# smann95/mpmc

Measured on AMD Instinct MI355X. Metric: MC steps/sec (polarizable, 4096 atoms), higher is better.
Workload: dtype f64; 1 GPU; PCN-61 cell + 416 BSSP H2, 4096 atoms (2016 frozen), polarizable, Jacobi x4, rc 8 A, FH4; energy() incremental (bit-identical to full); n_atoms=4096, n_polarizable=3264, n_atoms_final=4096, n_polarizable_final=3264, walkers=1, parallelism=1 independent walkers, 1 per GPU, collective=none (single walker, no launcher), rccl_ranks=1

## Files before the change

include/mpmc_hip.h:

```cpp
#ifndef MPMC_HIP_H
#define MPMC_HIP_H

#include <stddef.h>
#include <stdint.h>

#ifdef __cplusplus
extern "C" {
#endif

#define MPMC_HIP_ABI_VERSION 1

typedef struct mpmc_hip_ctx mpmc_hip_ctx;
typedef struct mpmc_hip_comm mpmc_hip_comm;

typedef struct mpmc_hip_params {
    double temperature;
    int rd_only;
    int rd_lrc;
    int feynman_hibbs;
    int feynman_hibbs_order;
    int ewald_alpha_set;
    double ewald_alpha;
    int ewald_kmax;
    int polarization;
// ... 18 lines not shown

typedef struct mpmc_hip_result {
    double energy;
    double rd_energy;
    double coulombic_energy;
    double polarization_energy;
    double es_real, es_recip, es_self;
    double dipole_rrms;
    double volume, cutoff, ewald_alpha, polar_ewald_alpha;
    int polar_iterations;
    int iter_success;
    int n_atoms;
    int status;
} mpmc_hip_result;

typedef struct mpmc_hip_timings {
    float pair_ms;
    float recip_ms;
    float field_ms;
    float amatrix_ms;
    float sweep_ms;
    float palmo_ms;
    float other_ms;
    float total_ms;
    int sweep_count;
    int amatrix_count;
    int graph_steps;
    float event_pair_ms;
    int event_pair_count;
    int spec_rank_redos;
    int resident_calls;
    int resident_fallbacks;
    int pending_sweeps;
} mpmc_hip_timings;

const char *mpmc_hip_last_error(void);
int mpmc_hip_abi_version(void);
int mpmc_hip_device_count(void);

int mpmc_hip_create(mpmc_hip_ctx **ctx, int device, int max_atoms);
void mpmc_hip_destroy(mpmc_hip_ctx *ctx);

int mpmc_hip_set_option(mpmc_hip_ctx *ctx, const char *name, int value);

void mpmc_hip_default_params(mpmc_hip_params *p);
int mpmc_hip_set_params(mpmc_hip_ctx *ctx, const mpmc_hip_params *p);

int mpmc_hip_set_box(mpmc_hip_ctx *ctx, const double basis[9], double pbc_cutoff);

int mpmc_hip_scale_box(mpmc_hip_ctx *ctx, const double basis[9], double pbc_cutoff,
                       int n_molecules, const double *delta );

int mpmc_hip_upload(mpmc_hip_ctx *ctx, int n, const double *x, const double *y, const double *z,
                    const double *charge, const double *polarizability, const double *epsilon,
                    const double *sigma, const double *mass, const int *molecule, const uint8_t *frozen);

typedef struct mpmc_hip_disp_params {
    int disp_expansion;
    int damp_dispersion;
    int extrapolate_disp_coeffs;
    int schmidt_mixing;
} mpmc_hip_disp_params;

int mpmc_hip_set_dispersion(mpmc_hip_ctx *ctx, const mpmc_hip_disp_params *p, int n, const double *c6, const double *c8,
                            const double *c10);

// ... 40 lines not shown
int mpmc_hip_cavity_bin(mpmc_hip_ctx *ctx, int n, const double *x, const double *y, const double *z);
int mpmc_hip_cavity_update(mpmc_hip_ctx *ctx, int n_out, const double *out_xyz, int n_in, const double *in_xyz,
                           int n_darts, const double *dart_xyz, int *cavities_open, int *hits);
int mpmc_hip_cavity_point(mpmc_hip_ctx *ctx, int index, int *grid_index, double pos[3]);
int mpmc_hip_download_cavity_grid(mpmc_hip_ctx *ctx, int *occupancy, double *pos);

int mpmc_hip_update_atoms(mpmc_hip_ctx *ctx, int first, int count, const double *x, const double *y,
                          const double *z);

int mpmc_hip_insert_molecule(mpmc_hip_ctx *ctx, int count, const double *x, const double *y, const double *z,
                             const double *charge, const double *polarizability, const double *epsilon,
                             const double *sigma, const double *mass, int frozen, int *first_slot);
int mpmc_hip_remove_molecule(mpmc_hip_ctx *ctx, int first_slot, int count);

typedef struct {
    int count;
    int frozen;
    const double *x, *y, *z, *charge, *polarizability, *epsilon, *sigma, *mass;
    const double *c6, *c8, *c10;
    const double *c9;
} mpmc_hip_molecule;

int mpmc_hip_edit_molecules(mpmc_hip_ctx *ctx,
                            int nremove, const int *remove_first_slot, const int *remove_count,
                            int ninsert, const mpmc_hip_molecule *insert, int *insert_first_slot);
int mpmc_hip_set_sweep_order(mpmc_hip_ctx *ctx, int count, const int *slots);
int mpmc_hip_slot_count(mpmc_hip_ctx *ctx);

int mpmc_hip_energy(mpmc_hip_ctx *ctx, mpmc_hip_result *out);

int mpmc_hip_energy_begin(mpmc_hip_ctx *ctx);
int mpmc_hip_energy_end(mpmc_hip_ctx *ctx, mpmc_hip_result *out);

int mpmc_hip_download_dipoles(mpmc_hip_ctx *ctx, double *mu, double *ef_static, double *ef_induced,
                              double *ef_induced_change);

int mpmc_hip_download_amatrix(mpmc_hip_ctx *ctx, double *A);

int mpmc_hip_download_ranking(mpmc_hip_ctx *ctx, double *rank_metric, int *ranked_array);

int mpmc_hip_get_timings(mpmc_hip_ctx *ctx, mpmc_hip_timings *t);

int mpmc_hip_comm_unique_id(unsigned char id[128]);
int mpmc_hip_comm_create(mpmc_hip_comm **comm, mpmc_hip_ctx *ctx, int nranks, int rank,
                         const unsigned char id[128]);
int mpmc_hip_comm_size(const mpmc_hip_comm *comm);
int mpmc_hip_comm_rank(const mpmc_hip_comm *comm);
int mpmc_hip_allreduce_observables(mpmc_hip_comm *comm, double *values, int count);
int mpmc_hip_allreduce_observables_begin(mpmc_hip_comm *comm, const double *values, int count);
int mpmc_hip_allreduce_observables_end(mpmc_hip_comm *comm, double *values);
int mpmc_hip_gather_observables(mpmc_hip_comm *comm, const void *record, int bytes, void *records);
void mpmc_hip_comm_destroy(mpmc_hip_comm *comm);

#ifdef __cplusplus
}
#endif
#endif
```

mpmc_amd/csrc/device_common.h:

```cpp
#pragma once
#include <hip/hip_runtime.h>
#include <stdint.h>

#include "step_pods.h"

namespace mpmc {

constexpr double kHBAR2 = 1.11211999e-68;
constexpr double kHBAR4 = 1.23681087e-136;
constexpr double kKB = 1.3806503e-23;
constexpr double kKB2 = 1.90619525e-46;
constexpr double kM2A2 = 1.0e20;
constexpr double kM2A4 = 1.0e40;
constexpr double kAMU2KG = 1.66053873e-27;
constexpr double kDEBYE2SKA = 85.10597636;
constexpr double kMAXVALUE = 1.0e40;
constexpr double kSMALL_dR = 1.0e-12;
constexpr int kMAX_ITERATION_COUNT = 128;
constexpr double kPI = 3.14159265358979323846;
constexpr double kOneOverSqrtPi = 0.56418958354;

constexpr int kWave = 64;

enum AtomFlag : int { kFrozen = 1, kValid = 2 };

struct DevBox {
    double b[3][3];
    double rb[3][3];
    double cutoff;
    double volume;
    float fb[3][3];
    float frb[3][3];
    float rc2_pre;
    int screen64;
    float half_tie32;
    double tie64;
    int tie_guard;
};

constexpr int kMaxMoves = 32;
struct MoveList {
    int n;
    int idx[kMaxMoves];
    double x[kMaxMoves], y[kMaxMoves], z[kMaxMoves];
};
struct MoveTargets {
    double *x, *y, *z;
    const int *slot_of_atom;
    double *px, *py, *pz;
};

struct DevAtoms {
    const double *x, *y, *z;
    const double *q, *alpha, *eps, *sig, *molmass;
    const int *mol;
    const int *flags;
    int n, npad;
};

__device__ __forceinline__ void moved_position(const DevAtoms &a, const MoveList &m, int i, double &x, double &y,
                                               double &z) {
    x = a.x[i];
    y = a.y[i];
    z = a.z[i];
    for (int e = 0; e < m.n; ++e) {
        if (m.idx[e] == i) {
            x = m.x[e];
            y = m.y[e];
            z = m.z[e];
        }
    }
}

__device__ __forceinline__ void minimum_image(const DevBox &bx, double dx, double dy, double dz, double &r,
                                              double &rimg, double &ox, double &oy, double &oz) {
#pragma clang fp contract(off)
    double i0 = bx.rb[0][0] * dx;
    i0 = i0 + bx.rb[1][0] * dy;
// ... 154 lines not shown
```

mpmc_amd/csrc/engine.hip:

```cpp
#include "../../include/mpmc_hip.h"

#include <dlfcn.h>
#include <hip/hip_runtime.h>
#include <hip/hip_ext.h>
#include <rccl/rccl.h>

#include <algorithm>
#include <cmath>
#include <cstdarg>
#include <cstdio>
#include <cstring>
#include <map>
#include <memory>
#include <tuple>
#include <utility>
#include <ctime>
#include <numeric>
#include <atomic>
#include <string>
#include <vector>

#include "device_common.h"
#include "step_plan.h"
#include "kernels_pair.h"
// ... 216 lines not shown
    int timing_interval = 32;
    int persistent_gs = 1;
    int spec_rank = 1;
    int fuse_tensor = 1;
    int gs_lags = 3;
    int gs_build_fork = 1;
    int gs_side_waves = 0;
    int rank_view_side = 1;
    int gs_fold_upper = 1;
    int gs_fold_finish = 1;
    int rank_late = 1;
    int resident = 1;
    int res_fold = 16;
    int res_side = 0;
    int sweep_alternate = 1;
    int sweep_nt = -1;
    int sweep_split = -1;
    int fuse_moves = 1;
    int gs_fuse_moves = 1;
    int fuse_field = 1;
    int fuse_recip = 1;
    int split_record = 1;
    int side_moves = 1;
    int res_stamps = 0;
    int sweep_ablate = 0;
    int res_fault = 0;
    int gs_stamps = 0;
    int inv_stamps = 0;
    int gs_ablate = 0;
    int gs_fault_sweep = 0;
    int graph = 0;
};

struct CallState {
    bool do_polar = false;
    bool gs_mode = false;
    bool exact = false;
    bool two_streams = false;
    bool plain_launches = false;
    DirtyBlocks dirty_blocks;
    DirtyBlocks lrc_blocks;
    bool lrc_edited = false;
    bool pair_part_valid_before = false;
    bool moves_deferred = false;
    bool moves_in_pair = false;
    bool side_carry = false;
    MoveList side_moves;
    MoveList pair_moves;
    MoveList side_apply;
    bool side_applied = false;
    bool coef_job_valid = false;
    bool coef_job_fork = false;
    CoefJob coef_job;
    bool build_join_pending = false;
    bool rank_on_side = false;
    int gs_sweeps = 0;
    bool gs_used[2] = {false, false};
    bool polar_first = false;
    bool side_open = false;
    bool side_done = false;
    int side_rc = 0;
    bool may_publish_early = false;
    bool published = false;
    int publish_rc = 0;
    bool recip_fused = false;
    int recip_chunks = 0;
    int pair_rows_to_sum = 0;
    unsigned res_zero_mask = 0;
    bool split = false;
    bool resident = false;
    bool spec_rank = false;
    bool timed = false;
    int iterations = 0, iter_success = 0;
};

struct TileSum {
    DevBuf<double> part;
    bool valid = false;
};

struct mpmc_hip_ctx {
    int device = 0;
    int num_cus = 256;
    int max_atoms = 0, max_npad = 0;
    int n = 0, npad = 0;
    EngineOptions opt;
// ... 120 lines not shown
    DevBuf<double> d_recipsum;
    bool self_valid = false;
    double self_alpha = 0.0;
    DevBuf<KVecF> d_kvecf;
    DevBuf<double2> d_sf;
    int nkf = 0;
    double kvecf_alpha = -1.0;
    int kvecf_kmax = -1;
    bool kvecf_valid = false;
    DevBuf<double> d_rank;
    DevBuf<double> d_rankpart;
    DevBuf<double> d_rank_used;
    DevBuf<unsigned int> d_rankcnt;
    std::vector<double> rank_saved;
    bool perm_ranked = false;
    bool rank_used_valid = false;
    bool force_host_rank = false;
    unsigned long long spec_redos = 0;
    int n_valid = 0;
    int next_mol = 0;
    std::vector<char> slot_valid;
    std::vector<char> slot_polar;
    std::vector<std::pair<int, int>> holes;
    std::vector<int> lrc_dirty_atoms;
    int n_mol_uploaded = 0;
    bool edited = false;
    bool order_stale = false;
    bool resident_off = false;
    long resident_retry_at = 0;
    long resident_backoff = 0;
    bool force_multi_launch = false;
    bool res_attr_set = false;
    unsigned long long resident_calls = 0, resident_fallbacks = 0;
    int graph_mode = 0;
    StepGraph sg;
    int eligible_streak = 0;
    unsigned long long graph_launches = 0;
    double graph_update_s = 0.0, graph_launch_s = 0.0;
    PinnedBuf<int> h_dirty;
    PinnedBuf<double> h_stage;
    size_t stage_used = 0;
    DevBuf<double> d_delta;
    DevBuf<double> d_res;
    PinnedBuf<double> h_res;
    double *h_res_dev = nullptr;
    PinnedBuf<double> h_res2;
    double *h_res2_dev = nullptr;
    PinnedBuf<unsigned long long> h_err;
    PinnedBuf<unsigned> h_gserr;
    PinnedBuf<int> h_order;
    PinnedBuf<double> h_rank;
    PinnedBuf<int> h_perm;
    PinnedBuf<int> h_slotmap;
    std::vector<HipEvent> ev_pool;
    size_t ev_next = 0;
    std::vector<TimeRec> recs;
    HipEvent ev_first, ev_last;
    bool timed = false;
    double host_enqueue_s = 0.0, host_wait_s = 0.0;
};

static DevAtoms dev_atoms(const mpmc_hip_ctx *c) {
    DevAtoms a;
    a.x = c->d_x;
    a.y = c->d_y;
    a.z = c->d_z;
// ... 43 lines not shown
}

static int thole_model_of(const mpmc_hip_ctx *c) {
    if (c->thole_damp_type == 0) return kTholeOff;
    if (c->thole_damp_type == 1) return kTholeLinear;
    return c->thole_wolf_full ? kTholeExpWolf : kTholeExp;
}
static TholeParams thole_params(const mpmc_hip_ctx *c, const int *idx) {
    TholeParams tp;
    tp.damp = c->par.polar_damp;
    tp.rc = c->cutoff;
    tp.irc3 = tp.wdamp1 = tp.wdamp2 = 0.0;
    tp.idx = nullptr;
    const int model = thole_model_of(c);
    if (model == kTholeOff) tp.idx = idx;
    if (model == kTholeExpWolf) {
        const double l = tp.damp, l2 = l * l, l3 = l2 * l, rc = tp.rc, rc2 = rc * rc, rc3 = rc2 * rc;
        const double explrcut = std::exp(-l * rc);
        tp.wdamp1 = 1.0 - explrcut * (0.5 * l2 * rc2 + l * rc + 1.0);
        tp.wdamp2 = tp.wdamp1 - explrcut * (l3 * rc3 / 6.0);
        tp.irc3 = 1.0 / rc3;
    }
    return tp;
}
#define MPMC_THOLE_DISPATCH(c, ...)                                                   \
    do switch (thole_model_of(c)) {                                                   \
        case kTholeLinear: { constexpr int kM = kTholeLinear; __VA_ARGS__; break; }   \
        case kTholeOff: { constexpr int kM = kTholeOff; __VA_ARGS__; break; }         \
        case kTholeExpWolf: { constexpr int kM = kTholeExpWolf; __VA_ARGS__; break; } \
        default: { constexpr int kM = kTholeExp; __VA_ARGS__; break; }                \
    } while (0)

static int complete_pending_sweep(mpmc_hip_ctx *c);
template <int NRHS>
static int exact_substitute(mpmc_hip_ctx *c, int nv, int nvpad, const double *es);
static void drop_polar_result(mpmc_hip_ctx *c) {
    c->psweep.drop();
    c->have_polar_result = false;
}
static void (*chain_kernel_of(int ortho))(GsChain);

static void note_coords(mpmc_hip_ctx *c, const double *x, const double *y, const double *z, int count) {
    double m = c->coord_max;
    for (int i = 0; i < count; ++i) {
        const double v = std::max(std::fabs(x[i]), std::max(std::fabs(y[i]), std::fabs(z[i])));
        if (!(v <= m)) m = (v == v) ? v : INFINITY;
    }
    const bool was64 = c->coord_max > kScreen32MaxCoord;
    c->coord_max = m;
    if ((m > kScreen32MaxCoord) != was64) ++c->config_rev;
}

static inline bool is_timed_call(const mpmc_hip_ctx *c) {
    return c->opt.timing >= 2 || ((c->opt.timing == 1 || c->opt.timing == -1) &&
                                 (c->energy_calls % (unsigned long long)c->opt.timing_interval) == 0ull);
}

template <typename... KArgs, typename... Args, size_t... I>
static hipError_t launch_slot_impl(mpmc_hip_ctx *c, int slot, void (*kernel)(KArgs...), dim3 g, dim3 b, hipStream_t s,
                                   std::index_sequence<I...>, Args &&...args) {
    std::tuple<KArgs...> vals(std::forward<Args>(args)...);
    void *argv[] = {(void *)&std::get<I>(vals)...};
    if (c->graph_mode == GM_UPDATE) {
        hipKernelNodeParams p;
        memset(&p, 0, sizeof(p));
        p.func = (void *)kernel;
// ... 101 lines not shown
         c->opt.resident = v;
         if (v) c->resident_off = false;
         return 0;
     }},
    {"resident_fold", &EngineOptions::res_fold, nullptr},
    {"resident_side", &EngineOptions::res_side, nullptr},
    {"sweep_alternate", &EngineOptions::sweep_alternate, nullptr},
    {"sweep_nt", &EngineOptions::sweep_nt, nullptr},
    {"sweep_split", &EngineOptions::sweep_split, nullptr},
    {"fuse_moves", &EngineOptions::fuse_moves, nullptr},
    {"gs_fuse_moves", &EngineOptions::gs_fuse_moves, nullptr},
    {"fuse_field", &EngineOptions::fuse_field, nullptr},
    {"fuse_recip", &EngineOptions::fuse_recip, nullptr},
    {"split_record", &EngineOptions::split_record, nullptr},
    {"side_moves", &EngineOptions::side_moves, nullptr},
    {"resident_stamps", &EngineOptions::res_stamps, nullptr},
    {"sweep_ablate", &EngineOptions::sweep_ablate, nullptr},
    {"resident_fault", &EngineOptions::res_fault, nullptr},
    {"gs_stamps", &EngineOptions::gs_stamps, nullptr},
    {"inv_stamps", &EngineOptions::inv_stamps, nullptr},
    {"gs_ablate", &EngineOptions::gs_ablate, nullptr},
    {"gs_fault_sweep", &EngineOptions::gs_fault_sweep, nullptr},
    {"step_graph", &EngineOptions::graph, nullptr},
};

extern "C" int mpmc_hip_set_option(mpmc_hip_ctx *c, const char *name, int value) {
    if (!c || !name) return fail("MPMC_HIP: set_option: null argument");
    if (!strcmp(name, "cavity_incremental")) {
        c->cav_incremental = value;
        return 0;
    }
    if (complete_pending_sweep(c)) return -1;
    ++c->config_rev;
    for (const OptionRow &o : kOptions) {
        if (strcmp(name, o.name)) continue;
        if (o.hook) return o.hook(c, value);
        c->opt.*o.member = value;
        return 0;
    }
    return fail("MPMC_HIP: set_option: unknown option '%s'", name);
}

extern "C" void mpmc_hip_default_params(mpmc_hip_params *p) {
    memset(p, 0, sizeof(*p));
    p->rd_lrc = 1;
    p->ewald_kmax = 7;
    p->polar_gamma = 1.0;
    p->polar_max_iter = 10;
    p->feynman_hibbs_order = 2;
}

extern "C" int mpmc_hip_create(mpmc_hip_ctx **out, int device, int max_atoms) {
    if (!out || max_atoms <= 0) return fail("MPMC_HIP: create: bad arguments");
    int ndev = 0;
    if (hipGetDeviceCount(&ndev) != hipSuccess || ndev <= 0)
        return fail("MPMC_HIP: no HIP device available (this engine has no CPU fallback)");
    if (device < 0 || device >= ndev) return fail("MPMC_HIP: device %d out of range (%d present)", device, ndev);
    (void)hipSetDeviceFlags(hipDeviceScheduleSpin);
    HIPCHK(hipSetDevice(device));
    hipDeviceProp_t prop;
    HIPCHK(hipGetDeviceProperties(&prop, device));
    if (strncmp(prop.gcnArchName, "gfx950", 6) != 0)
        return fail("MPMC_HIP: device %d is %s; this engine is built for gfx950 (MI355X) only", device,
                    prop.gcnArchName);
    std::unique_ptr<mpmc_hip_ctx> owner(new mpmc_hip_ctx());
    mpmc_hip_ctx *c = owner.get();
// ... 87 lines not shown
    HIPCHK(hipHostGetDevicePointer((void **)&c->h_res_dev, c->h_res, 0));
    HIPCHK(c->h_res2.alloc(R_COUNT + 1, hipHostMallocMapped));
    memset(c->h_res2, 0, (R_COUNT + 1) * sizeof(double));
    HIPCHK(hipHostGetDevicePointer((void **)&c->h_res2_dev, c->h_res2, 0));
    HIPCHK(c->h_err.alloc(1));
    HIPCHK(c->h_gserr.alloc(2));
    HIPCHK(c->h_rank.alloc(np));
    HIPCHK(c->h_perm.alloc(np));
    HIPCHK(c->h_slotmap.alloc(np));
    HIPCHK(c->h_dirty.alloc(kMaxDirty));
    HIPCHK(c->h_stage.alloc(3 * 4096));
    c->ev_pool.resize(2 * 512);
    for (auto &e : c->ev_pool) HIPCHK(hipEventCreate(e.out()));
    HIPCHK(hipEventCreate(c->ev_first.out()));
    HIPCHK(hipEventCreate(c->ev_last.out()));
    HIPCHK(hipMemsetAsync(c->d_res, 0, R_COUNT * sizeof(double), c->stream));
    HIPCHK(hipStreamSynchronize(c->stream));
    if (device < 64) ++g_ctx_on_device[device];
    *out = owner.release();
    return 0;
}

static void graph_destroy(mpmc_hip_ctx *c);

extern "C" void mpmc_hip_destroy(mpmc_hip_ctx *c) {
    if (!c) return;
    if (getenv("MPMC_HIP_HOST_PROFILE") && c->energy_calls)
        fprintf(stderr, "MPMC_HIP host profile: %llu energy() calls (%llu as graph), enqueue %.1f us, wait %.1f us per call\n",
                c->energy_calls, c->graph_launches, 1e6 * c->host_enqueue_s / c->energy_calls,
                1e6 * c->host_wait_s / c->energy_calls);
    if (getenv("MPMC_HIP_HOST_PROFILE") && c->graph_launches)
        fprintf(stderr, "MPMC_HIP graph steps: node updates %.1f us, launch %.1f us per step\n",
                1e6 * c->graph_update_s / c->graph_launches, 1e6 * c->graph_launch_s / c->graph_launches);
    hipSetDevice(c->device);
    hipStreamSynchronize(c->stream);
    hipStreamSynchronize(c->stream2);
    hipStreamSynchronize(c->stream3);
    graph_destroy(c);
    if (c->device < 64) --g_ctx_on_device[c->device];
    delete c;
}

static void positions_unknown(mpmc_hip_ctx *c) {
    c->pair_part_valid = c->field_part_valid = c->disp.valid = c->rdc.valid = c->at.valid = false;
    c->rep.valid = c->vdw.valid = c->rdf.valid = false;
}
static void params_or_grid_changed(mpmc_hip_ctx *c) {
    c->pair_part_valid = c->field_part_valid = c->disp.valid = c->rdc.valid = false;
    c->rep.valid = c->vdw.valid = false;
    c->rdf.valid = false;
}
static void grid_grew(mpmc_hip_ctx *c) {
    params_or_grid_changed(c);
    c->lrc.valid = c->disp_lrc.valid = c->rdf_lrc.valid = c->rdc_static.valid = c->at.valid = false;
}
static void box_changed(mpmc_hip_ctx *c) {
    c->lrc.valid = c->disp_lrc.valid = c->rdc_static.valid = c->rep_lrc.valid = c->vdw_lrc.valid = false;
    c->rdf_lrc.valid = false;
    c->cav_pos_valid = c->cav_occ_valid = false;
    c->cav_open = -1;
}
static void atoms_replaced(mpmc_hip_ctx *c) {
    c->lrc.valid = c->disp.valid = c->disp_lrc.valid = c->at.valid = c->rdc.valid = c->rdc_static.valid = false;
    c->rep.valid = c->rep_lrc.valid = c->vdw.valid = c->vdw_lrc.valid = false;
    c->rdf.valid = c->rdf_lrc.valid = false;
}
// ... 66 lines not shown
    memcpy(c->basis, b, sizeof(b));
    memcpy(c->recip, rb, sizeof(rb));
    c->pbc_cutoff_in = pbc_cutoff;
    c->cutoff = cutoff;
    c->volume = vol;
    c->have_box = true;
    ++c->config_rev;
    c->box_ortho = (b[0][1] == 0.0 && b[0][2] == 0.0 && b[1][0] == 0.0 && b[1][2] == 0.0 && b[2][0] == 0.0 &&
                    b[2][1] == 0.0);
    c->kvecf_valid = false;
    c->kvec_valid = false;
    box_changed(c);
    c->all_dirty = true;
    return 0;
}

extern "C" int mpmc_hip_set_box(mpmc_hip_ctx *c, const double basis[9], double pbc_cutoff) {
    if (!c || !basis) return fail("MPMC_HIP: set_box: null argument");
    if (c->in_flight) return fail("MPMC_HIP: set_box between energy_begin() and energy_end()");
    if (complete_pending_sweep(c)) return -1;
    return apply_box(c, basis, pbc_cutoff);
}

extern "C" int mpmc_hip_upload(mpmc_hip_ctx *c, int n, const double *x, const double *y, const double *z,
                               const double *charge, const double *polarizability, const double *epsilon,
                               const double *sigma, const double *mass, const int *molecule,
                               const uint8_t *frozen) {
    if (!c) return fail("MPMC_HIP: upload: null context");
    if (c->in_flight) return fail("MPMC_HIP: upload between energy_begin() and energy_end()");
    if (n <= 0 || n > c->max_atoms) return fail("MPMC_HIP: upload: n = %d outside (0, %d]", n, c->max_atoms);
    if (!x || !y || !z || !charge || !polarizability || !epsilon || !sigma || !mass || !molecule || !frozen)
        return fail("MPMC_HIP: upload: null array");
    HIPCHK(hipSetDevice(c->device));
    drop_polar_result(c);
    const int npad = round_up(n, 128);
    const int nall = c->max_npad;
    std::vector<double> hx(nall, 0.0), hy(nall, 0.0), hz(nall, 0.0), hq(nall, 0.0), ha(nall, 0.0), he(nall, 0.0),
        hs(nall, 0.0), hm(nall, 0.0);
    std::vector<int> hmol(nall, -1), hfl(nall, 0);
    int m = -1;
    for (int i = 0; i < n; ++i) {
        if (i == 0 || molecule[i] != molecule[i - 1]) ++m;
        hmol[i] = m;
        hx[i] = x[i];
        hy[i] = y[i];
        hz[i] = z[i];
        hq[i] = charge[i];
        ha[i] = polarizability[i];
        he[i] = epsilon[i];
        hs[i] = sigma[i];
        hfl[i] = kValid | (frozen[i] ? kFrozen : 0);
    }
    for (int s = 0; s < n;) {
        int e = s;
        double mm = 0.0;
        while (e < n && hmol[e] == hmol[s]) mm += mass[e++];
        for (int i = s; i < e; ++i) hm[i] = mm;
        s = e;
    }
    for (int i = n; i < nall; ++i) hmol[i] = -2 - i;
    const size_t bd = nall * sizeof(double), bi = nall * sizeof(int);
    HIPCHK(hipMemcpyAsync(c->d_x, hx.data(), bd, hipMemcpyHostToDevice, c->stream));
    HIPCHK(hipMemcpyAsync(c->d_y, hy.data(), bd, hipMemcpyHostToDevice, c->stream));
    HIPCHK(hipMemcpyAsync(c->d_z, hz.data(), bd, hipMemcpyHostToDevice, c->stream));
    HIPCHK(hipMemcpyAsync(c->d_q, hq.data(), bd, hipMemcpyHostToDevice, c->stream));
    HIPCHK(hipMemcpyAsync(c->d_alpha, ha.data(), bd, hipMemcpyHostToDevice, c->stream));
    HIPCHK(hipMemcpyAsync(c->d_eps, he.data(), bd, hipMemcpyHostToDevice, c->stream));
    HIPCHK(hipMemcpyAsync(c->d_sig, hs.data(), bd, hipMemcpyHostToDevice, c->stream));
    HIPCHK(hipMemcpyAsync(c->d_molmass, hm.data(), bd, hipMemcpyHostToDevice, c->stream));
    HIPCHK(hipMemcpyAsync(c->d_mol, hmol.data(), bi, hipMemcpyHostToDevice, c->stream));
    HIPCHK(hipMemcpyAsync(c->d_flags, hfl.data(), bi, hipMemcpyHostToDevice, c->stream));
    HIPCHK(hipStreamSynchronize(c->stream));
    c->coord_max = 0.0;
    note_coords(c, x, y, z, n);
    c->n = n;
    c->npad = npad;
    c->n_valid = n;
    c->next_mol = m + 1;
    c->n_mol_uploaded = m + 1;
    c->edited = false;
    c->slot_valid.assign(n, 1);
    c->slot_polar.assign(n, 0);
    for (int i = 0; i < n; ++i) c->slot_polar[i] = (polarizability[i] != 0.0);
    c->holes.clear();
    c->lrc_dirty_atoms.clear();
    c->self_valid = false;
    c->have_atoms = true;
    c->have_polar_result = false;
    c->disp_on = false;
    c->at_on = false;
    c->chol_nv = 0;
    c->vdw_on = false;
    c->negative_sigma = false;
    for (int i = 0; i < n; ++i) c->negative_sigma = c->negative_sigma || sigma[i] < 0.0;
    atoms_replaced(c);
    c->rank_saved.clear();
    c->perm_ranked = false;
    c->pending.n = 0;
    SweepView &v0 = c->view[0];
    v0.h_idx.clear();
    for (int i = 0; i < n; ++i)
        if (polarizability[i] != 0.0) v0.h_idx.push_back(i);
    v0.nv = (int)v0.h_idx.size();
    v0.nvpad = std::max(128, round_up(v0.nv, 128));
    v0.slot_of_atom.assign(n, -1);
    for (int k = 0; k < v0.nv; ++k) v0.slot_of_atom[v0.h_idx[k]] = k;
    {
// ... 12 lines not shown
    c->rank_used_valid = false;
    c->order_stale = false;
    c->view[0].rebuild_from = c->view[1].rebuild_from = -1;
    ++c->config_rev;
    if (v0.nv > 0) HIPCHK(hipMemcpy(v0.d_idx, v0.h_idx.data(), v0.nv * sizeof(int), hipMemcpyHostToDevice));
    return 0;
}

static int flush_moves(mpmc_hip_ctx *c);
static int alloc_zero_params(mpmc_hip_ctx *c) {
    if (c->d_zero) return 0;
    HIPCHK(c->d_zero.alloc(c->max_npad));
    HIPCHK(hipMemsetAsync(c->d_zero, 0, (size_t)c->max_npad * sizeof(double), c->stream));
    HIPCHK(hipStreamSynchronize(c->stream));
    return 0;
}
static int per_atom_setter_refused(const mpmc_hip_ctx *c, const char *name) {
    if (c->in_flight) return fail("MPMC_HIP: %s between energy_begin() and energy_end()", name);
    if (!c->have_atoms) return fail("MPMC_HIP: %s: no configuration uploaded", name);
    if (c->edited) return fail("MPMC_HIP: %s: molecules were inserted or removed since the upload", name);
    return 0;
}
static void lj_kernels_switched(mpmc_hip_ctx *c) {
    c->pair_part_valid = c->lrc.valid = false;
    c->all_dirty = true;
    ++c->config_rev;
}
extern "C" int mpmc_hip_set_dispersion(mpmc_hip_ctx *c, const mpmc_hip_disp_params *p, int n, const double *c6,
                                       const double *c8, const double *c10) {
    if (!c || !p) return fail("MPMC_HIP: set_dispersion: null argument");
    if (per_atom_setter_refused(c, "set_dispersion")) return -1;
    if (n != c->n) return fail("MPMC_HIP: set_dispersion: %d coefficients for the %d atoms of the upload", n, c->n);
    HIPCHK(hipSetDevice(c->device));
    if (flush_moves(c)) return -1;
    c->disp.valid = c->disp_lrc.valid = false;
    lj_kernels_switched(c);
    if (!p->disp_expansion) {
        c->disp_on = false;
        return 0;
    }
    if (!c6 || !c8 || !c10) return fail("MPMC_HIP: set_dispersion: null array");
    const size_t nall = c->max_npad, ntile = nall / 64;
    if (!c->d_c6) {
        HIPCHK(c->d_c6.alloc(nall));
        HIPCHK(c->d_c8.alloc(nall));
        HIPCHK(c->d_c10.alloc(nall));
        HIPCHK(c->disp.part.alloc(ntile * ntile));
        HIPCHK(c->disp_lrc.part.alloc(ntile * ntile));
    }
    if (alloc_zero_params(c)) return -1;
    std::vector<double> h6(nall, 0.0), h8(nall, 0.0), h10(nall, 0.0);
    std::copy(c6, c6 + n, h6.begin());
    std::copy(c8, c8 + n, h8.begin());
    std::copy(c10, c10 + n, h10.begin());
    const size_t bd = nall * sizeof(double);
    HIPCHK(hipMemcpyAsync(c->d_c6, h6.data(), bd, hipMemcpyHostToDevice, c->stream));
    HIPCHK(hipMemcpyAsync(c->d_c8, h8.data(), bd, hipMemcpyHostToDevice, c->stream));
    HIPCHK(hipMemcpyAsync(c->d_c10, h10.data(), bd, hipMemcpyHostToDevice, c->stream));
    HIPCHK(hipStreamSynchronize(c->stream));
    c->disp_par.damp = p->damp_dispersion != 0;
    c->disp_par.extrapolate = p->extrapolate_disp_coeffs != 0;
    c->disp_par.schmidt = p->schmidt_mixing != 0;
    c->disp_on = true;
    return 0;
}

static void at_site_values(double alpha, double c9, double &a, double &g) {
    a = alpha * kAtAlpha;
    g = (a != 0.0) ? 1.0 / (c9 / std::pow(a, 3)) : 1.0;
}

extern "C" int mpmc_hip_set_axilrod_teller(mpmc_hip_ctx *c, int enable, int n, const double *c9) {
    if (!c) return fail("MPMC_HIP: set_axilrod_teller: null context");
    if (per_atom_setter_refused(c, "set_axilrod_teller")) return -1;
    HIPCHK(hipSetDevice(c->device));
    if (!enable) {
        if (flush_moves(c)) return -1;
        c->at_on = false;
        c->at.valid = false;
        ++c->config_rev;
        return 0;
    }
    if (n != c->n) return fail("MPMC_HIP: set_axilrod_teller: %d coefficients for the %d atoms of the upload", n, c->n);
    if (!c9) return fail("MPMC_HIP: set_axilrod_teller: null array");
    if (flush_moves(c)) return -1;
    const size_t nall = c->max_npad;
    std::vector<double> ha(nall, 0.0), hg(nall, 1.0);
    HIPCHK(hipMemcpyAsync(ha.data(), c->d_alpha, (size_t)n * sizeof(double), hipMemcpyDeviceToHost, c->stream));
    HIPCHK(hipStreamSynchronize(c->stream));
    for (int i = 0; i < n; ++i) {
        const double alpha = ha[i];
        if (alpha < 0.0) return fail("MPMC_HIP: set_axilrod_teller: negative polarizability %g of atom %d", alpha, i);
        at_site_values(alpha, c9[i], ha[i], hg[i]);
    }
    if (!c->d_at_a) {
        HIPCHK(c->d_at_a.alloc(nall));
        HIPCHK(c->d_at_g.alloc(nall));
        HIPCHK(c->at.part.alloc((size_t)at_unit_count((int)(nall / 64)) * kAtSplit));
    }
    const size_t bd = nall * sizeof(double);
    HIPCHK(hipMemcpyAsync(c->d_at_a, ha.data(), bd, hipMemcpyHostToDevice, c->stream));
    HIPCHK(hipMemcpyAsync(c->d_at_g, hg.data(), bd, hipMemcpyHostToDevice, c->stream));
    HIPCHK(hipStreamSynchronize(c->stream));
    c->at.valid = false;
    c->at_on = true;
    ++c->config_rev;
    return 0;
}

extern "C" int mpmc_hip_set_rd_crystal(mpmc_hip_ctx *c, int order) {
    if (!c) return fail("MPMC_HIP: set_rd_crystal: null context");
    if (c->in_flight) return fail("MPMC_HIP: set_rd_crystal between energy_begin() and energy_end()");
    if (order < 0 || order > kRdcMaxOrder)
        return fail("MPMC_HIP: set_rd_crystal: rd_crystal_order %d outside 1 .. %d (0 = off)", order, kRdcMaxOrder);
    if (order == c->rdc_order) return 0;
    HIPCHK(hipSetDevice(c->device));
    if (c->have_atoms && flush_moves(c)) return -1;
    if (order > 0) {
        const size_t ntile = c->max_npad / 64;
        if (alloc_zero_params(c)) return -1;
        if (!c->rdc.part) {
            HIPCHK(c->rdc.part.alloc(ntile * ntile));
            HIPCHK(c->rdc_static.part.alloc(ntile * ntile));
        }
    }
    c->rdc_order = order;
    c->rdc.valid = c->rdc_static.valid = false;
    c->pair_part_valid = false;
    c->lrc.valid = false;
    c->all_dirty = true;
    ++c->config_rev;
    return 0;
}

extern "C" int mpmc_hip_set_rd_form(mpmc_hip_ctx *c, const mpmc_hip_rd_form_params *p) {
    if (!c || !p) return fail("MPMC_HIP: set_rd_form: null argument");
    if (c->in_flight) return fail("MPMC_HIP: set_rd_form between energy_begin() and energy_end()");
    if (p->form < 0 || p->form > MPMC_HIP_RD_BUFFERED_14_7)
        return fail("MPMC_HIP: set_rd_form: form %d outside 0 .. %d", p->form, MPMC_HIP_RD_BUFFERED_14_7);
    if (p->mixing < 0 || p->mixing > MPMC_HIP_RD_MIX_C6)
        return fail("MPMC_HIP: set_rd_form: mixing %d outside 0 .. %d", p->mixing, MPMC_HIP_RD_MIX_C6);
    const int mix = p->form ? p->mixing : 0;
    if (p->form == c->rd_form && mix == c->rd_mix) return 0;
    HIPCHK(hipSetDevice(c->device));
    if (complete_pending_sweep(c)) return -1;
// ... 61 lines not shown
}

extern "C" int mpmc_hip_get_polarizability_tensor(mpmc_hip_ctx *c, double out[9]) {
    if (!c || !out) return fail("MPMC_HIP: get_polarizability_tensor: null argument");
    if (c->in_flight) return fail("MPMC_HIP: get_polarizability_tensor between energy_begin() and energy_end()");
    if (!c->exact_polar)
        return fail("MPMC_HIP: get_polarizability_tensor: the exact dipoles are off (mpmc_hip_set_exact_polar; the reference: "
                    "iterative polarizability tensor method not implemented)");
    if (c->chol_nv <= 0 || !c->chol_done)
        return fail("MPMC_HIP: get_polarizability_tensor: no energy() with polarization has completed in this mode");
    if (c->chol_failed)
        return fail("MPMC_HIP: get_polarizability_tensor: the matrix of the last energy() was not positive definite");
    HIPCHK(hipSetDevice(c->device));
    if (exact_substitute<3>(c, c->chol_nv, c->chol_nvpad, nullptr)) return -1;
    hipLaunchKernelGGL(chol_tensor_kernel, dim3(1), dim3(256), 0, c->stream, c->chol_nv,
                       (const double *)(c->d_chol_vec + 6 * (size_t)(3 * c->chol_nvpad)), 3 * c->chol_nvpad,
                       c->d_chol_tensor.get());
    HIPCHK(hipMemcpyAsync(out, c->d_chol_tensor, 9 * sizeof(double), hipMemcpyDeviceToHost, c->stream));
    HIPCHK(hipStreamSynchronize(c->stream));
    return 0;
}

extern "C" int mpmc_hip_get_three_body_energy(mpmc_hip_ctx *c, double *out) {
    if (!c || !out) return fail("MPMC_HIP: get_three_body_energy: null argument");
    if (c->in_flight) return fail("MPMC_HIP: get_three_body_energy between energy_begin() and energy_end()");
    *out = c->at_on ? c->three_body : 0.0;
    return 0;
}

extern "C" int mpmc_hip_set_vdw(mpmc_hip_ctx *c, int enable, int n, const double *omega, const int *mol_type) {
    if (!c) return fail("MPMC_HIP: set_vdw: null context");
    if (per_atom_setter_refused(c, "set_vdw")) return -1;
    HIPCHK(hipSetDevice(c->device));
    if (!enable) {
        c->vdw_iso.clear();
        if (!c->vdw_on) return 0;
        if (flush_moves(c)) return -1;
        c->vdw_on = false;
        c->rep.valid = c->rep_lrc.valid = c->vdw.valid = c->vdw_lrc.valid = false;
        lj_kernels_switched(c);
        return 0;
    }
    if (n != c->n) return fail("MPMC_HIP: set_vdw: %d frequencies for the %d atoms of the upload", n, c->n);
    if (!omega || !mol_type) return fail("MPMC_HIP: set_vdw: null array");
    if (flush_moves(c)) return -1;
    const size_t nall = c->max_npad, ntile = nall / 64;
    std::vector<double> ha(nall, 0.0), hw(nall, 0.0), hk;
    std::vector<int> hmol(nall, 0), hidx;
    HIPCHK(hipMemcpyAsync(ha.data(), c->d_alpha, (size_t)n * sizeof(double), hipMemcpyDeviceToHost, c->stream));
    HIPCHK(hipMemcpyAsync(hmol.data(), c->d_mol, (size_t)n * sizeof(int), hipMemcpyDeviceToHost, c->stream));
    HIPCHK(hipStreamSynchronize(c->stream));
    std::vector<mpmc_hip_ctx::VdwMolecule> mols;
    for (int i = 0; i < n; ++i) {
        if (ha[i] < 0.0) return fail("MPMC_HIP: set_vdw: negative polarizability %g of atom %d", ha[i], i);
        if (i == 0 || hmol[i] != hmol[i - 1]) {
            mols.push_back({mol_type[i], (int)hidx.size(), 0});
        } else if (mol_type[i] != mols.back().type) {
            return fail("MPMC_HIP: set_vdw: atom %d has type id %d, its molecule %d", i, mol_type[i], mols.back().type);
        }
        hw[i] = omega[i];
        const double k = std::sqrt(ha[i]) * omega[i];
        if (k != 0.0) {
            hidx.push_back(i);
            hk.push_back(k);
            ++mols.back().sites;
        }
// ... 18 lines not shown
        HIPCHK(hipMemcpyAsync(c->d_vdw_idx, hidx.data(), (size_t)na * sizeof(int), hipMemcpyHostToDevice, c->stream));
        HIPCHK(hipMemcpyAsync(c->d_vdw_k, hk.data(), (size_t)na * sizeof(double), hipMemcpyHostToDevice, c->stream));
    }
    HIPCHK(hipStreamSynchronize(c->stream));
    c->vdw_na = na;
    c->vdw_mols = std::move(mols);
    c->vdw_iso_summed = false;
    c->rep.valid = c->rep_lrc.valid = c->vdw.valid = c->vdw_lrc.valid = false;
    if (c->vdw_on)
        ++c->config_rev;
    else
        lj_kernels_switched(c);
    c->vdw_on = true;
    return 0;
}

extern "C" int mpmc_hip_get_vdw_energy(mpmc_hip_ctx *c, double *out) {
    if (!c || !out) return fail("MPMC_HIP: get_vdw_energy: null argument");
    if (c->in_flight) return fail("MPMC_HIP: get_vdw_energy between energy_begin() and energy_end()");
    *out = c->vdw_on ? c->vdw_energy : 0.0;
    return 0;
}

extern "C" int mpmc_hip_get_vdw_terms(mpmc_hip_ctx *c, double terms[5]) {
    if (!c || !terms) return fail("MPMC_HIP: get_vdw_terms: null argument");
    if (c->in_flight) return fail("MPMC_HIP: get_vdw_terms between energy_begin() and energy_end()");
    for (int k = 0; k < 5; ++k) terms[k] = c->vdw_on ? c->vdw_terms[k] : 0.0;
    return 0;
}

extern "C" int mpmc_hip_set_autoreject(mpmc_hip_ctx *c, double scale) {
    if (!c) return fail("MPMC_HIP: set_autoreject: null context");
    if (c->in_flight) return fail("MPMC_HIP: set_autoreject between energy_begin() and energy_end()");
    if (!(scale >= 0.0) || !std::isfinite(scale)) return fail("MPMC_HIP: set_autoreject: scale %g (0 = off)", scale);
    if (scale == c->autoreject_scale) return 0;
    HIPCHK(hipSetDevice(c->device));
    if (c->have_atoms && flush_moves(c)) return -1;
    c->autoreject_scale = scale;
    c->pair_part_valid = false;
    c->all_dirty = true;
    ++c->config_rev;
    return 0;
}

extern "C" int mpmc_hip_get_close_contacts(mpmc_hip_ctx *c, long long *count) {
    if (!c || !count) return fail("MPMC_HIP: get_close_contacts: null argument");
    if (c->in_flight) return fail("MPMC_HIP: get_close_contacts between energy_begin() and energy_end()");
    *count = c->autoreject_scale != 0.0 ? c->close_contacts : 0;
    return 0;
}

static void side_wait_for_moves(mpmc_hip_ctx *c, hipStream_t s);
static void feed_side_stream(mpmc_hip_ctx *c);
static void publish_early(mpmc_hip_ctx *c);
static int flush_moves(mpmc_hip_ctx *c) {
    if (c->pending.n > 0) {
        if (complete_pending_sweep(c)) return -1;
        SweepView &v0 = c->view[0];
        HIPCHK(launch_slot(c, GS_MOVES, apply_moves_kernel, dim3(1), dim3(64), c->stream, c->pending, c->d_x, c->d_y,
                           c->d_z, v0.d_slot, v0.px, v0.py, v0.pz));
        c->pending.n = 0;
    }
    return 0;
}

static void side_wait_for_moves(mpmc_hip_ctx *c, hipStream_t s) {
    if (c->call.side_apply.n > 0) {
        SweepView &v0 = c->view[0];
        hipLaunchKernelGGL(apply_moves_kernel, dim3(1), dim3(64), 0, s, c->call.side_apply, c->d_x, c->d_y, c->d_z,
                           (const int *)v0.d_slot, v0.px, v0.py, v0.pz);
        c->call.side_apply.n = 0;
        c->call.side_applied = true;
        return;
    }
    if (c->call.side_applied) return;
    hipStreamWaitEvent(s, c->ev_fork, 0);
}

extern "C" int mpmc_hip_update_atoms(mpmc_hip_ctx *c, int first, int count, const double *x, const double *y,
                                     const double *z) {
    if (!c || !c->have_atoms) return fail("MPMC_HIP: update_atoms: no configuration uploaded");
    if (c->in_flight) return fail("MPMC_HIP: update_atoms between energy_begin() and energy_end()");
    if (first < 0 || count <= 0 || first + count > c->n)
        return fail("MPMC_HIP: update_atoms: range [%d, %d) outside [0, %d)", first, first + count, c->n);
    if (!x || !y || !z) return fail("MPMC_HIP: update_atoms: null array");
    HIPCHK(hipSetDevice(c->device));
    note_coords(c, x, y, z, count);
    const size_t b = count * sizeof(double);
    bool queued = false;
    if (count <= kMaxMoves) {
        MoveList &m = c->pending;
        int need = 0;
        for (int i = 0; i < count; ++i) {
            bool found = false;
            for (int k = 0; k < m.n; ++k) found |= (m.idx[k] == first + i);
            need += !found;
        }
        if (m.n + need <= kMaxMoves) {
            for (int i = 0; i < count; ++i) {
                int slot = -1;
                for (int k = 0; k < m.n; ++k)
                    if (m.idx[k] == first + i) slot = k;
                if (slot < 0) slot = m.n++;
                m.idx[slot] = first + i;
                m.x[slot] = x[i];
                m.y[slot] = y[i];
                m.z[slot] = z[i];
            }
            queued = true;
        }
    }
    if (queued) {
    } else if ((size_t)(3 * count) <= c->h_stage.size()) {
        if (complete_pending_sweep(c)) return -1;
        if (flush_moves(c)) return -1;
        c->staged_copies = true;
        c->main_writes = true;
        c->view[0].pos_valid = false;
        if (c->stage_used + 3 * (size_t)count > c->h_stage.size()) {
            HIPCHK(hipStreamSynchronize(c->stream));
// ... 29 lines not shown

extern "C" int mpmc_hip_scale_box(mpmc_hip_ctx *c, const double basis[9], double pbc_cutoff, int n_molecules,
                                  const double *delta) {
    if (!c || !basis || !delta) return fail("MPMC_HIP: scale_box: null argument");
    if (c->in_flight) return fail("MPMC_HIP: scale_box between energy_begin() and energy_end()");
    if (!c->have_atoms || !c->have_box) return fail("MPMC_HIP: scale_box: no configuration uploaded");
    if (c->edited || !c->holes.empty()) return 1;
    if (n_molecules != c->n_mol_uploaded)
        return fail("MPMC_HIP: scale_box: %d displacements for the %d molecules of the upload", n_molecules,
                    c->n_mol_uploaded);
    HIPCHK(hipSetDevice(c->device));
    const size_t need = 3 * (size_t)n_molecules;
    double dmax = 0.0;
    for (size_t k = 0; k < need; ++k) {
        const double v = std::fabs(delta[k]);
        if (!(v <= dmax)) dmax = (v == v) ? v : INFINITY;
    }
    if (complete_pending_sweep(c)) return -1;
    if (flush_moves(c)) return -1;
    if (c->d_delta.size() < need) {
        HIPCHK(hipStreamSynchronize(c->stream));
        HIPCHK(c->d_delta.alloc(need));
    }
    if (c->h_stage.size() < 2 * need) {
        HIPCHK(hipStreamSynchronize(c->stream));
        HIPCHK(c->h_stage.alloc(2 * need + 3 * 4096));
        c->stage_used = 0;
    }
    if (c->stage_used + need > c->h_stage.size()) {
        HIPCHK(hipStreamSynchronize(c->stream));
        c->stage_used = 0;
    }
    if (apply_box(c, basis, pbc_cutoff)) return -1;
    double *s = c->h_stage + c->stage_used;
    memcpy(s, delta, need * sizeof(double));
    c->stage_used += need;
    HIPCHK(hipMemcpyAsync(c->d_delta, s, need * sizeof(double), hipMemcpyHostToDevice, c->stream));
    SweepView &v0 = c->view[0];
    hipLaunchKernelGGL(shift_molecules_kernel, dim3((c->n + kShiftThreads - 1) / kShiftThreads), dim3(kShiftThreads), 0,
                       c->stream, c->n, n_molecules, (const double *)c->d_delta, (const int *)c->d_mol,
                       (const int *)c->d_flags, c->d_x.get(), c->d_y.get(), c->d_z.get(), (const int *)v0.d_slot,
                       v0.px.get(), v0.py.get(), v0.pz.get());
    HIPCHK(hipGetLastError());
    {
        const bool was64 = c->coord_max > kScreen32MaxCoord;
        double bound = c->coord_max + dmax;
        if (!was64 && bound > kScreen32MaxCoord) {
            hipLaunchKernelGGL(coord_absmax_kernel, dim3(1), dim3(kShiftThreads), 0, c->stream, c->n,
                               (const int *)c->d_flags, (const double *)c->d_x, (const double *)c->d_y,
                               (const double *)c->d_z, c->d_delta.get());
            double truth = INFINITY;
            HIPCHK(hipMemcpyAsync(&truth, c->d_delta, sizeof(double), hipMemcpyDeviceToHost, c->stream));
            HIPCHK(hipStreamSynchronize(c->stream));
            c->stage_used = 0;
            bound = truth;
        }
        c->coord_max = bound;
        if ((c->coord_max > kScreen32MaxCoord) != was64) ++c->config_rev;
    }
    c->staged_copies = true;
    c->main_writes = true;
    c->dirty_atoms.clear();
    for (SweepView &v : c->view) v.A_valid = v.C_valid = false;
    c->view[1].pos_valid = false;
    c->rank_used_valid = false;
    c->rank_saved.clear();
// ... 21 lines not shown
    if (c->exact_polar) return false;
    if (!P.rd_only && P.polarization && (P.polar_gs || P.polar_gs_ranked) && !gs_order_mode(c)) return false;
    return true;
}

static int launch_edits(mpmc_hip_ctx *c, const EditList &ed) {
    SweepView &v0 = c->view[0];
    EditTargets t;
    t.x = c->d_x;
    t.y = c->d_y;
    t.z = c->d_z;
    t.q = c->d_q;
    t.alpha = c->d_alpha;
    t.eps = c->d_eps;
    t.sig = c->d_sig;
    t.molmass = c->d_molmass;
    t.mol = c->d_mol;
    t.flags = c->d_flags;
    t.slot_of_atom = v0.d_slot;
    t.idx_of_slot = v0.d_idx;
    t.px = v0.px;
    t.py = v0.py;
    t.pz = v0.pz;
    t.palpha = v0.palpha;
    t.pflags = v0.pflags;
    t.c6 = c->disp_on ? c->d_c6.get() : nullptr;
    t.c8 = c->disp_on ? c->d_c8.get() : nullptr;
    t.c10 = c->disp_on ? c->d_c10.get() : nullptr;
    t.at_a = c->at_on ? c->d_at_a.get() : nullptr;
    t.at_g = c->at_on ? c->d_at_g.get() : nullptr;
    drop_polar_result(c);
    if (flush_moves(c)) return -1;
    c->main_writes = true;
    hipLaunchKernelGGL(apply_edits_kernel, dim3(1), dim3(64), 0, c->stream, ed, t);
    HIPCHK(hipGetLastError());
    return 0;
}

static void mark_edited(mpmc_hip_ctx *c, int first, int count) {
    for (int i = 0; i < count; ++i) {
        c->dirty_atoms.push_back(first + i);
        c->lrc_dirty_atoms.push_back(first + i);
    }
    if ((int)c->dirty_atoms.size() > 4 * kMaxDirty) c->all_dirty = true;
    c->have_polar_result = false;
    c->self_valid = false;
    c->rank_used_valid = false;
    c->edited = true;
    ++c->config_rev;
}

extern "C" int mpmc_hip_slot_count(mpmc_hip_ctx *c) { return c ? c->n : 0; }

struct DenseAtomData {
    const double *c6 = nullptr, *c8 = nullptr, *c10 = nullptr;
    const double *c9 = nullptr;
};
static int remove_checked(mpmc_hip_ctx *c, int first, int count);
static int insert_checked(mpmc_hip_ctx *c, int count, const double *x, const double *y, const double *z, const double *charge,
                          const double *polarizability, const double *epsilon, const double *sigma, const double *mass,
                          int frozen, const DenseAtomData &dd, int *first_slot);

static int new_view_slots(const mpmc_hip_ctx *c, int first, int count, const double *polarizability) {
    return count_new_view_slots(c->view[0].slot_of_atom, gs_order_mode(c), first, count, polarizability);
}

extern "C" int mpmc_hip_remove_molecule(mpmc_hip_ctx *c, int first, int count) {
    if (!c || !c->have_atoms) return fail("MPMC_HIP: remove_molecule: no configuration uploaded");
    if (c->in_flight) return fail("MPMC_HIP: remove_molecule between energy_begin() and energy_end()");
    if (first < 0 || count <= 0 || first + count > c->n)
        return fail("MPMC_HIP: remove_molecule: range [%d, %d) outside [0, %d)", first, first + count, c->n);
    for (int i = 0; i < count; ++i)
        if (!c->slot_valid[first + i]) return fail("MPMC_HIP: remove_molecule: slot %d holds no atom", first + i);
    if (count > kMaxEdit || !edits_supported(c)) return 1;
    return remove_checked(c, first, count);
}

static int remove_checked(mpmc_hip_ctx *c, int first, int count) {
    HIPCHK(hipSetDevice(c->device));
    SweepView &v0 = c->view[0];
    EditList ed;
    memset(&ed, 0, sizeof(ed));
    ed.n = count;
    for (int i = 0; i < count; ++i) {
        ed.idx[i] = first + i;
        ed.at_g[i] = 1.0;
        ed.vslot[i] = gs_order_mode(c) ? -1 : v0.slot_of_atom[first + i];
        ed.mol[i] = -2 - (first + i);
        ed.flags[i] = 0;
        c->slot_valid[first + i] = 0;
        c->slot_polar[first + i] = 0;
    }
    if (launch_edits(c, ed)) return -1;
    c->holes.push_back(std::make_pair(first, count));
    c->n_valid -= count;
    mark_edited(c, first, count);
    if (gs_order_mode(c)) {
        c->order_stale = true;
        v0.pos_valid = false;
    }
    return 0;
}

extern "C" int mpmc_hip_insert_molecule(mpmc_hip_ctx *c, int count, const double *x, const double *y, const double *z,
                                        const double *charge, const double *polarizability, const double *epsilon,
                                        const double *sigma, const double *mass, int frozen, int *first_slot) {
    if (!c || !c->have_atoms) return fail("MPMC_HIP: insert_molecule: no configuration uploaded");
    if (c->in_flight) return fail("MPMC_HIP: insert_molecule between energy_begin() and energy_end()");
    if (count <= 0 || !x || !y || !z || !charge || !polarizability || !epsilon || !sigma || !mass || !first_slot)
        return fail("MPMC_HIP: insert_molecule: bad arguments");
    if (count > kMaxEdit || !edits_supported(c)) return 1;
    HIPCHK(hipSetDevice(c->device));
    note_coords(c, x, y, z, count);
    int first, hole;
    if (!place_molecule(c->holes, c->n, c->max_atoms, count, first, hole)) return 1;
    if (c->view[0].nv + new_view_slots(c, first, count, polarizability) > c->view[0].cap) return 1;
    return insert_checked(c, count, x, y, z, charge, polarizability, epsilon, sigma, mass, frozen, DenseAtomData(), first_slot);
}

static int insert_checked(mpmc_hip_ctx *c, int count, const double *x, const double *y, const double *z, const double *charge,
                          const double *polarizability, const double *epsilon, const double *sigma, const double *mass,
                          int frozen, const DenseAtomData &dd, int *first_slot) {
    SweepView &v0 = c->view[0];
    int first, hole;
    place_molecule(c->holes, c->n, c->max_atoms, count, first, hole);
    const bool gs_mode = gs_order_mode(c);
    if (hole >= 0)
        c->holes.erase(c->holes.begin() + hole);
    else {
        c->n += count;
        c->slot_valid.resize(c->n, 0);
        c->slot_polar.resize(c->n, 0);
        v0.slot_of_atom.resize(c->n, -1);
        const int npad = round_up(c->n, 128);
        if (npad != c->npad) {
            c->npad = npad;
            grid_grew(c);
        }
    }
    double mm = 0.0;
    for (int i = 0; i < count; ++i) mm += mass[i];
// ... 23 lines not shown
        ed.sig[i] = sigma[i];
        ed.molmass[i] = mm;
        if (dd.c6) {
            ed.c6[i] = dd.c6[i];
            ed.c8[i] = dd.c8[i];
            ed.c10[i] = dd.c10[i];
        }
        ed.at_g[i] = 1.0;
        if (dd.c9) at_site_values(polarizability[i], dd.c9[i], ed.at_a[i], ed.at_g[i]);
        c->slot_valid[a] = 1;
        c->slot_polar[a] = (polarizability[i] != 0.0);
    }
    const int nvpad = std::max(128, round_up(v0.nv, 128));
    if (nvpad != v0.nvpad) {
        v0.nvpad = nvpad;
        v0.A_valid = false;
    }
    if (launch_edits(c, ed)) return -1;
    c->n_valid += count;
    mark_edited(c, first, count);
    if (gs_mode) {
        c->order_stale = true;
        v0.pos_valid = false;
    }
    *first_slot = first;
    return 0;
}

constexpr int kMaxEditMolecules = 8;
extern "C" int mpmc_hip_edit_molecules(mpmc_hip_ctx *c, int nremove, const int *remove_first_slot, const int *remove_count,
                                       int ninsert, const mpmc_hip_molecule *insert, int *insert_first_slot) {
    if (!c || !c->have_atoms) return fail("MPMC_HIP: edit_molecules: no configuration uploaded");
    if (c->in_flight) return fail("MPMC_HIP: edit_molecules between energy_begin() and energy_end()");
    if (nremove < 0 || ninsert < 0 || (nremove > 0 && (!remove_first_slot || !remove_count)) ||
        (ninsert > 0 && (!insert || !insert_first_slot)))
        return fail("MPMC_HIP: edit_molecules: bad arguments");
    if (nremove > kMaxEditMolecules || ninsert > kMaxEditMolecules) return 1;
    std::vector<char> leaving(c->n, 0);
    size_t atoms = 0;
    bool too_large = false;
    for (int r = 0; r < nremove; ++r) {
        const int first = remove_first_slot[r], count = remove_count[r];
        if (first < 0 || count <= 0 || count > c->n || first > c->n - count)
            return fail("MPMC_HIP: edit_molecules: removal %d: range [%d, %d + %d) outside [0, %d)", r, first, first, count, c->n);
        for (int i = 0; i < count; ++i) {
            if (!c->slot_valid[first + i] || leaving[first + i])
                return fail("MPMC_HIP: edit_molecules: removal %d: slot %d holds no atom", r, first + i);
            leaving[first + i] = 1;
        }
        too_large = too_large || count > kMaxEdit;
        atoms += count;
    }
    for (int m = 0; m < ninsert; ++m) {
        const mpmc_hip_molecule &M = insert[m];
        if (M.count <= 0 || !M.x || !M.y || !M.z || !M.charge || !M.polarizability || !M.epsilon || !M.sigma || !M.mass)
            return fail("MPMC_HIP: edit_molecules: insertion %d: bad arguments", m);
        if (c->disp_on && (!M.c6 || !M.c8 || !M.c10))
            return fail("MPMC_HIP: edit_molecules: c6 / c8 / c10 missing while disp_expansion is on (insertion %d)", m);
        if (c->at_on && !M.c9) return fail("MPMC_HIP: edit_molecules: c9 missing while axilrod_teller is on (insertion %d)", m);
        too_large = too_large || M.count > kMaxEdit;
        if (M.count > kMaxEdit) continue;
        if (c->at_on)
            for (int i = 0; i < M.count; ++i)
                if (M.polarizability[i] < 0.0)
                    return fail("MPMC_HIP: edit_molecules: negative polarizability %g under axilrod_teller (insertion %d, atom %d)",
                                M.polarizability[i], m, i);
// ... 11 lines not shown
            if (hole >= 0)
                holes.erase(holes.begin() + hole);
            else
                n += insert[m].count;
            new_view += new_view_slots(c, first, insert[m].count, insert[m].polarizability);
        }
        if (c->view[0].nv + new_view > c->view[0].cap) return 1;
    }
    HIPCHK(hipSetDevice(c->device));
    for (int r = 0; r < nremove; ++r)
        if (remove_checked(c, remove_first_slot[r], remove_count[r])) return -1;
    for (int m = 0; m < ninsert; ++m) {
        const mpmc_hip_molecule &M = insert[m];
        note_coords(c, M.x, M.y, M.z, M.count);
        for (int i = 0; i < M.count; ++i)
            if (M.sigma[i] < 0.0) c->negative_sigma = true;
        DenseAtomData dd;
        if (c->disp_on) {
            dd.c6 = M.c6;
            dd.c8 = M.c8;
            dd.c10 = M.c10;
        }
        if (c->at_on) dd.c9 = M.c9;
        if (insert_checked(c, M.count, M.x, M.y, M.z, M.charge, M.polarizability, M.epsilon, M.sigma, M.mass, M.frozen, dd,
                           &insert_first_slot[m]))
            return -1;
    }
    return 0;
}

extern "C" int mpmc_hip_set_sweep_order(mpmc_hip_ctx *c, int count, const int *slots) {
    if (!c || !c->have_atoms) return fail("MPMC_HIP: set_sweep_order: no configuration uploaded");
    if (c->in_flight) return fail("MPMC_HIP: set_sweep_order between energy_begin() and energy_end()");
    if (!gs_order_mode(c)) return 0;
    SweepView &v0 = c->view[0];
    if (count < 0 || count > v0.cap || (count > 0 && !slots)) return fail("MPMC_HIP: set_sweep_order: bad arguments");
    std::vector<char> seen(c->n, 0);
    for (int k = 0; k < count; ++k) {
        const int a = slots[k];
        if (a < 0 || a >= c->n || !c->slot_valid[a] || seen[a])
            return fail("MPMC_HIP: set_sweep_order: entry %d (slot %d) is not a distinct atom of the configuration", k, a);
        if (!c->slot_polar[a])
            return fail("MPMC_HIP: set_sweep_order: entry %d (slot %d) is not a polarizable site", k, a);
        seen[a] = 1;
    }
    {
        int npolar = 0;
        for (int a = 0; a < c->n; ++a) npolar += (c->slot_valid[a] && c->slot_polar[a]);
        if (count != npolar)
            return fail("MPMC_HIP: set_sweep_order: %d slots stated, the configuration has %d polarizable sites", count, npolar);
    }
    HIPCHK(hipSetDevice(c->device));
    drop_polar_result(c);
    if (flush_moves(c)) return -1;
    c->main_writes = true;
    int p0 = 0;
    {
        const int m = std::min((int)v0.h_idx.size(), count);
        while (p0 < m && v0.h_idx[p0] == slots[p0]) ++p0;
    }
    const bool keep_prefix = v0.C_valid && v0.rebuild_from < 0 && v0.M_epoch == v0.C_epoch && v0.M_call == c->energy_calls;
    v0.h_idx.assign(slots, slots + count);
    v0.nv = count;
    v0.nvpad = std::max(128, round_up(count, 128));
    v0.slot_of_atom.assign(c->n, -1);
    if (!c->h_order) {
// ... 119 lines not shown
    (void)c;
    const int ntld = std::max(nt, (v.cap + kCoefTile - 1) / kCoefTile);
    const size_t need = (size_t)ntld * ntld * kCoefTile * kCoefTile;
    if (v.C.size() < need || v.ntld != ntld) {
        HIPCHK(v.C.alloc(need));
        HIPCHK(hipMemsetAsync(v.C, 0, need * sizeof(double2), st));
        v.ntld = ntld;
        v.C_valid = false;
    }
    return 0;
}

static int ensure_view_chain(mpmc_hip_ctx *c, SweepView &v, hipStream_t st) {
    if (v.Minv && v.Lnb_lags >= c->opt.gs_lags) return 0;
    const size_t nbcap = (size_t)(v.cap + 63) / 64;
    for (; v.Lnb_lags < c->opt.gs_lags; ++v.Lnb_lags) {
        HIPCHK(v.Lnb[v.Lnb_lags].alloc(nbcap * kPnbDoubles));
        v.M_epoch = 0;
    }
    if (v.Minv) return 0;
    HIPCHK(v.Minv.alloc(nbcap * kMinvDoubles));
    HIPCHK(hipMemsetAsync(v.Minv, 0, nbcap * kMinvDoubles * sizeof(double), st));
    v.M_epoch = 0;
    return 0;
}

static int ensure_view_matrix(SweepView &v) {
    const size_t need = (size_t)(3 * (size_t)v.nvpad) * (3 * (size_t)v.nvpad);
    if (v.A.size() < need) HIPCHK(v.A.alloc(need));
    return 0;
}

static int ensure_static_field(mpmc_hip_ctx *c) {
    if (!c->es_stale) return 0;
    hipLaunchKernelGGL(field_reduce_kernel, dim3(c->npad / 64), dim3(64 * kFieldGroups), 0, c->stream, c->d_fieldpart,
                       c->es_slots, c->npad, c->d_es);
    c->es_stale = false;
    return 0;
}

template <int K>
constexpr int resident_lds_bytes() {
    return (int)std::max(sizeof(ResidentLds<K>), (size_t)kResFinisherLds);
}
constexpr int kResMaxK = 1;
constexpr int kResidentLdsOnePerCu = 84 * 1024;
constexpr int kResidentLdsMax = std::max(kResidentLdsOnePerCu, resident_lds_bytes<kResMaxK>());
static_assert(kResidentLdsMax <= 160 * 1024, "LDS of a CU");
typedef void (*ResidentKernel)(ResidentSolve);
static ResidentKernel resident_kernel_of(int ortho, int K, bool fold) {
    (void)K;
    if (fold) return ortho ? jacobi_folded_kernel<1> : jacobi_folded_kernel<0>;
    return ortho ? jacobi_resident_kernel<1, 1> : jacobi_resident_kernel<0, 1>;
}
static std::vector<const void *> resident_kernels() {
    std::vector<const void *> v;
    for (int o = 0; o < 2; ++o) {
        for (int K = 1; K <= kResMaxK; ++K) v.push_back(reinterpret_cast<const void *>(resident_kernel_of(o, K, false)));
        v.push_back(reinterpret_cast<const void *>(resident_kernel_of(o, 1, true)));
    }
    return v;
}

struct ResidentPlan {
    bool ok = false;
    bool fold = false;
// ... 737 lines not shown
        if (c->thole_damp_type != 2 || c->thole_wolf_full)
            return fail("MPMC_HIP: energy: polarvdw with polar_damp_type linear / off or polar_wolf_full "
                        "(mpmc_hip_set_thole_model) is not implemented (the reference's e2body() / calc_e_iso() are written "
                        "for the exponential form)");
        if (c->disp_on)
            return fail("MPMC_HIP: energy: polarvdw with disp_expansion (mpmc_hip_set_dispersion) is not implemented");
        if (c->rdc_order)
            return fail("MPMC_HIP: energy: polarvdw with rd_crystal (mpmc_hip_set_rd_crystal) is not implemented");
        if (c->at_on)
            return fail("MPMC_HIP: energy: polarvdw with axilrod_teller (mpmc_hip_set_axilrod_teller) is not implemented");
        if (c->par.feynman_hibbs)
            return fail("MPMC_HIP: energy: polarvdw with feynman_hibbs is not implemented (the reference's finite-difference "
                        "correction cannot be matched)");
    } else {
        c->vdw_iso.clear();
    }
    if (c->exact_polar && c->par.polarization && !c->par.rd_only) {
        if (c->par.polar_zodid)
            return fail("MPMC_HIP: energy: polar_zodid and polar_iterative are incompatible: the exact dipoles "
                        "(mpmc_hip_set_exact_polar) with polar_zodid are refused");
        if (c->par.polar_palmo)
            return fail("MPMC_HIP: energy: the exact dipoles (mpmc_hip_set_exact_polar) with polar_palmo are not implemented "
                        "(the reference would add a stale ef_induced_change)");
        if (c->vdw_on)
            return fail("MPMC_HIP: energy: the exact dipoles (mpmc_hip_set_exact_polar) with polarvdw (mpmc_hip_set_vdw) are not "
                        "implemented (the reference forces the iterative solver there)");
    } else if (c->par.polarization && !c->par.rd_only && !c->par.polar_zodid && c->par.polar_precision == 0.0 &&
               c->par.polar_max_iter <= 0) {
        return fail("MPMC_HIP: polar_max_iter must be > 0 when polar_precision is 0");
    }
    return 0;
}

extern "C" int mpmc_hip_energy_begin(mpmc_hip_ctx *c) {
    if (!c) return fail("MPMC_HIP: energy: null argument");
    if (c->in_flight) return fail("MPMC_HIP: energy_begin: the previous evaluation has not been collected");
    if (!c->have_atoms) return fail("MPMC_HIP: energy: no configuration uploaded");
    if (!c->have_box) return fail("MPMC_HIP: energy: no box set");
    if (c->order_stale && gs_order_mode(c))
        return fail("MPMC_HIP: energy: Gauss-Seidel after insert_molecule / remove_molecule needs the sweep order of the "
                    "new configuration (mpmc_hip_set_sweep_order)");
    if (const int rc = refuse_unsupported(c)) return rc;
    if (!c->exact_polar) c->chol_nv = 0;
    HIPCHK(hipSetDevice(c->device));
    if (c->vdw_on && !c->par.rd_only && vdw_ensure_iso(c)) return -1;
    if (c->resident_off && c->resident_backoff > 0 && (long)c->energy_calls >= c->resident_retry_at)
        c->resident_off = false;
    const mpmc_hip_params &P = c->par;
    c->ewald_alpha = P.ewald_alpha_set ? P.ewald_alpha : 3.5 / c->cutoff;
    c->polar_ewald_alpha = P.polar_ewald_alpha_set ? P.polar_ewald_alpha : 3.5 / c->cutoff;
    if (!P.rd_only && !P.wolf && (!c->kvec_valid || c->kvec_kmax != P.ewald_kmax)) {
        if (build_kvectors(c)) return -1;
        c->kvec_kmax = P.ewald_kmax;
    }
    timespec ts0, ts1;
    clock_gettime(CLOCK_MONOTONIC, &ts0);
    begin_call(c);
    bool issued = false;
    if (graph_eligible(c)) {
        if (c->sg.valid && c->sg.rev == c->config_rev) {
            if (graph_step(c)) return -1;
            issued = true;
        } else if (++c->eligible_streak >= 3) {
            graph_destroy(c);
            const MoveList saved = c->pending;
            bool ok = hipStreamBeginCapture(c->stream, hipStreamCaptureModeThreadLocal) == hipSuccess;
            if (ok) {
                c->graph_mode = GM_CAPTURE;
                const int rc = enqueue_direct(c);
                c->graph_mode = GM_DIRECT;
                hipGraph_t graph = nullptr;
                ok = (hipStreamEndCapture(c->stream, &graph) == hipSuccess) && rc == 0 && graph != nullptr;
                if (ok) ok = graph_finish_capture(c, graph);
                else if (graph) hipGraphDestroy(graph);
            }
            if (ok) {
                c->sg.valid = true;
                c->sg.rev = c->config_rev;
                c->sg.iterations = c->call.iterations;
                c->sg.result_view = c->result_view;
                c->sg.result_mu = c->result_mu;
                c->sg.psweep = c->psweep;
                c->sg.energy_part = c->energy_part;
                c->sg.energy_nt = c->energy_nt;
                c->sg.recip_chunks = c->call.recip_chunks;
                c->sg.res_zero_mask = c->call.res_zero_mask;
                c->sg.pair_rows_to_sum = c->call.pair_rows_to_sum;
                HIPCHK(hipGraphLaunch(c->sg.exec, c->stream));
                ++c->graph_launches;
                issued = true;
            } else {
                (void)hipGetLastError();
                graph_destroy(c);
                c->opt.graph = 0;
                c->pending = saved;
                c->call = CallState();
                collect_dirty_blocks(c);
            }
        }
    } else {
        c->eligible_streak = 0;
    }
    if (!issued && enqueue_direct(c)) return -1;
    c->staged_copies = false;
    c->main_writes = false;
    clock_gettime(CLOCK_MONOTONIC, &ts1);
    c->host_enqueue_s += (ts1.tv_sec - ts0.tv_sec) + 1e-9 * (ts1.tv_nsec - ts0.tv_nsec);
    c->dirty_atoms.clear();
    c->all_dirty = false;
    c->in_flight = true;
    return 0;
}

static int wait_sequence(volatile double *seq, double want, hipStream_t stream) {
    for (unsigned long long spins = 0; spins < 2000000000ull; ++spins) {
        if (*seq == want) return 0;
        if ((spins & 0xfffffull) == 0xfffffull && hipStreamQuery(stream) != hipErrorNotReady) break;
        __builtin_ia32_pause();
    }
    HIPCHK(hipStreamSynchronize(stream));
    return 0;
}

static int wait_record(mpmc_hip_ctx *c) {
    const double want = (double)c->energy_calls;
    if (wait_sequence(c->h_res + R_COUNT, want, c->stream)) return -1;
    return c->call.split ? wait_sequence(c->h_res2 + R_COUNT, want, c->stream2) : 0;
}

static int repeat_call(mpmc_hip_ctx *c, bool &flag) {
    flag = true;
    begin_call(c);
    const int rc = enqueue_direct(c);
    flag = false;
    return rc ? -1 : wait_record(c);
}

static void assemble_result(mpmc_hip_ctx *c, int iter_success, mpmc_hip_result *out) {
    const mpmc_hip_params &P = c->par;
    const bool do_polar = c->call.do_polar;
    const int polar_iterations = c->call.iterations;
    double r[R_COUNT];
    for (int k = 0; k < R_COUNT; ++k) r[k] = (c->call.split && ((kSideSlots >> k) & 1u)) ? c->h_res2[k] : c->h_res[k];
    const double rd = c->disp_on     ? (r[R_RD_PAIR] + r[R_LRC]) + (r[R_DISP] + r[R_DISP_LRC])
                      : c->rdc_order ? (r[R_RD_PAIR] + r[R_LRC]) + ((r[R_DISP] + r[R_RDC_SELF]) + r[R_DISP_LRC])
                      : c->vdw_on    ? (r[R_RD_PAIR] + r[R_LRC]) + (r[R_DISP] + r[R_DISP_LRC])
                      : c->rd_form   ? (r[R_RD_PAIR] + r[R_LRC]) + (r[R_DISP] + r[R_DISP_LRC])
                                     : r[R_RD_PAIR] + r[R_LRC];
    const double real = r[R_ES_REAL] - r[R_ES_INTRA];
    const bool ewald = !P.rd_only && !P.wolf;
    const double recip = ewald ? r[R_RECIP] * (4.0 * kPI / c->volume) : 0.0;
    const double self = ewald ? r[R_SELF] : 0.0;
    const double coul = P.rd_only ? 0.0 : real + recip + self;
    const double upol = do_polar ? r[R_UPOL] : 0.0;
    out->rd_energy = rd;
    out->es_real = P.rd_only ? 0.0 : real;
    out->es_recip = recip;
    out->es_self = self;
    out->coulombic_energy = coul;
    out->polarization_energy = upol;
    out->energy = rd + coul + upol;
    c->three_body = c->at_on ? r[R_AT] : 0.0;
    if (c->at_on) out->energy += c->three_body;
// ... 59 lines not shown
    HIPCHK(hipGetLastError());
    c->timed = timed_call;
    c->stage_used = 0;
    assemble_result(c, iter_success, out);
    return 0;
}

extern "C" int mpmc_hip_download_dipoles(mpmc_hip_ctx *c, double *mu, double *ef_static, double *ef_induced,
                                         double *ef_induced_change) {
    if (!c || !c->have_atoms) return fail("MPMC_HIP: download_dipoles: no configuration");
    if (!c->have_polar_result) return fail("MPMC_HIP: download_dipoles: no polarization energy evaluated yet");
    HIPCHK(hipSetDevice(c->device));
    if (ensure_static_field(c)) return -1;
    if (complete_pending_sweep(c)) return -1;
    if (!c->results_scattered) {
        SweepView *V = c->result_view;
        hipLaunchKernelGGL(scatter_results_kernel, dim3((c->npad + 255) / 256), dim3(256), 0, c->stream, c->npad,
                           V->d_slot, c->result_mu, V->efind, V->efchg, c->d_mu, c->d_efind, c->d_efchg);
        HIPCHK(hipStreamSynchronize(c->stream));
        c->results_scattered = true;
    }
    const size_t b = 3 * (size_t)c->n * sizeof(double);
    if (mu) HIPCHK(hipMemcpy(mu, c->d_mu, b, hipMemcpyDeviceToHost));
    if (ef_static) HIPCHK(hipMemcpy(ef_static, c->d_es, b, hipMemcpyDeviceToHost));
    if (ef_induced) HIPCHK(hipMemcpy(ef_induced, c->d_efind, b, hipMemcpyDeviceToHost));
    if (ef_induced_change) HIPCHK(hipMemcpy(ef_induced_change, c->d_efchg, b, hipMemcpyDeviceToHost));
    return 0;
}

extern "C" int mpmc_hip_download_amatrix(mpmc_hip_ctx *c, double *A) {
    if (!c || !c->have_atoms || !c->have_box || !A) return fail("MPMC_HIP: download_amatrix: no configuration");
    HIPCHK(hipSetDevice(c->device));
    const size_t n3 = 3 * (size_t)c->n, lda = 3 * (size_t)c->npad;
    if (flush_moves(c)) return -1;
    DevBuf<double> dA;
    HIPCHK(dA.alloc(lda * lda));
    MPMC_THOLE_DISPATCH(c, hipLaunchKernelGGL((build_amatrix_kernel<kM>), dim3(c->npad / 128, c->npad / kARows), dim3(64), 0,
                                              c->stream, dev_atoms(c), dev_box(c), thole_params(c, nullptr), dA, (int)lda));
    hipError_t e = hipMemcpy2DAsync(A, n3 * sizeof(double), dA, lda * sizeof(double), n3 * sizeof(double), n3,
                                    hipMemcpyDeviceToHost, c->stream);
    if (e == hipSuccess) e = hipStreamSynchronize(c->stream);
    if (e != hipSuccess) return fail("MPMC_HIP: download_amatrix: %s", hipGetErrorString(e));
    return 0;
}

extern "C" int mpmc_hip_download_ranking(mpmc_hip_ctx *c, double *rank_metric, int *ranked_array) {
    if (!c || !c->have_atoms) return fail("MPMC_HIP: download_ranking: no configuration");
    HIPCHK(hipSetDevice(c->device));
    if (rank_metric) HIPCHK(hipMemcpy(rank_metric, c->d_rank, c->n * sizeof(double), hipMemcpyDeviceToHost));
    if (ranked_array) {
        std::vector<int> perm(c->n);
        std::iota(perm.begin(), perm.end(), 0);
        const SweepView &v0 = c->view[0];
        if (gs_order_mode(c) && !c->order_stale && (int)v0.slot_of_atom.size() == c->n) {
            size_t k = 0;
            for (int a = 0; a < c->n && k < v0.h_idx.size(); ++a)
                if (v0.slot_of_atom[a] >= 0) perm[a] = v0.h_idx[k++];
        }
        if (c->perm_ranked && (int)c->rank_saved.size() == c->n) {
            const double *rk = c->rank_saved.data();
            std::stable_sort(perm.begin(), perm.end(), [rk](int x, int y) { return rk[x] > rk[y]; });
        }
        memcpy(ranked_array, perm.data(), c->n * sizeof(int));
    }
    return 0;
}
// ... 179 lines not shown
    *grid_index = (int)c->h_cav[CR_PICK_G];
    for (int p = 0; p < 3; ++p) pos[p] = c->h_cav[CR_PICK_X + p];
    return 0;
}

extern "C" int mpmc_hip_download_cavity_grid(mpmc_hip_ctx *c, int *occupancy, double *pos) {
    if (cavity_check(c, "download_cavity_grid")) return -1;
    if (!occupancy && !pos) return fail("MPMC_HIP: download_cavity_grid: null argument");
    const size_t P = (size_t)c->cav_P;
    if (occupancy) {
        if (!c->cav_occ_valid) return fail("MPMC_HIP: download_cavity_grid: no occupancy (mpmc_hip_cavity_bin) for this grid and box");
        HIPCHK(hipMemcpyAsync(occupancy, c->d_cav_occ, P * sizeof(int), hipMemcpyDeviceToHost, c->stream));
    }
    if (pos) {
        if (cavity_ensure_points(c)) return -1;
        std::vector<double> soa(3 * P);
        HIPCHK(hipMemcpyAsync(soa.data(), c->d_cav_pos, 3 * P * sizeof(double), hipMemcpyDeviceToHost, c->stream));
        HIPCHK(hipStreamSynchronize(c->stream));
        for (size_t g = 0; g < P; ++g)
            for (int p = 0; p < 3; ++p) pos[3 * g + p] = soa[p * P + g];
    }
    HIPCHK(hipStreamSynchronize(c->stream));
    return 0;
}

extern "C" int mpmc_hip_get_timings(mpmc_hip_ctx *c, mpmc_hip_timings *t) {
    if (!c || !t) return fail("MPMC_HIP: get_timings: null argument");
    memset(t, 0, sizeof(*t));
    t->graph_steps = (int)c->graph_launches;
    t->spec_rank_redos = (int)c->spec_redos;
    t->resident_calls = (int)c->resident_calls;
    t->resident_fallbacks = (int)c->resident_fallbacks;
    t->pending_sweeps = (int)c->psweep.sweeps.size();
    if (!c->timed) return 0;
    HIPCHK(hipSetDevice(c->device));
    float acc[T_NCLASS] = {0};
    int cnt[T_NCLASS] = {0};
    for (const TimeRec &r : c->recs) {
        float ms = 0.f;
        HIPCHK(hipEventSynchronize(r.b));
        HIPCHK(hipEventElapsedTime(&ms, r.a, r.b));
        acc[r.cls] += ms;
        cnt[r.cls]++;
    }
    t->pair_ms = acc[T_PAIR];
    t->recip_ms = acc[T_RECIP];
    t->field_ms = acc[T_FIELD];
    t->amatrix_ms = acc[T_AMAT];
    t->sweep_ms = acc[T_SWEEP];
    t->palmo_ms = acc[T_PALMO];
    t->other_ms = acc[T_OTHER];
    t->sweep_count = cnt[T_SWEEP];
    t->amatrix_count = cnt[T_AMAT];
    t->event_pair_ms = acc[T_EVPAIR];
    t->event_pair_count = cnt[T_EVPAIR];
    float tot = 0.f;
    HIPCHK(hipEventElapsedTime(&tot, c->ev_first, c->ev_last));
    t->total_ms = tot;
    return 0;
}

struct Rccl {
    void *h = nullptr;
    ncclResult_t (*GetUniqueId)(ncclUniqueId *) = nullptr;
    ncclResult_t (*CommInitRank)(ncclComm_t *, int, ncclUniqueId, int) = nullptr;
    ncclResult_t (*AllReduce)(const void *, void *, size_t, ncclDataType_t, ncclRedOp_t, ncclComm_t,
// ... 135 lines not shown
```

mpmc_amd/csrc/engine_polar.inc:

```
static constexpr bool kSweepSplitAuto = false;

static int launch_coef_job(mpmc_hip_ctx *c, const DevBox &bx) {
    if (!c->call.coef_job_valid) return 0;
    c->call.coef_job_valid = false;
    const CoefJob &cj = c->call.coef_job;
    MPMC_THOLE_DISPATCH(c, hipLaunchKernelGGL((update_coef_moves_kernel<kM>), dim3(cj.nt, cj.dm.n), dim3(64), 0, c->stream, cj.pa,
                                              bx, cj.tp, cj.dm, cj.ntld, cj.C, cj.m, cj.gx, cj.gy, cj.gz, cj.slot_of_atom, cj.px,
                                              cj.py, cj.pz));
    if (c->call.coef_job_fork) hipEventRecord(c->ev_fork, c->stream);
    return 0;
}

static int launch_field(mpmc_hip_ctx *c, const DevAtoms &a, const DevBox &bx) {
    const mpmc_hip_params &P = c->par;
    ScopedTimer t(c, T_FIELD);
    FieldParams fp;
    fp.wolf_alpha = P.polar_wolf_alpha;
    fp.cutoffterm = 0.0;
    const int ntile = c->npad / 64;
    const ChunkPlan cp = chunk_plan(c->npad, 4096);
    const int nchunk = cp.nchunk, chunk = cp.chunk;
    fp.chunk = chunk;
    const bool wolf = P.polar_wolf || c->thole_wolf_full;
    const int mode = P.polar_ewald ? kFieldEwald : (!wolf ? kFieldBare : (P.polar_wolf_alpha == 0.0 ? kFieldWolf0 : kFieldWolfA));
    const int key = mode * 1000003 + chunk;
    DirtyBlocks sel = c->call.dirty_blocks;
    const bool resident = c->field_part_valid && c->field_key == key;
    if (!resident) sel.n = 0;
    const bool skip = resident && sel.n == 0 && c->dirty_atoms.empty();
    dim3 grid = (sel.n > 0) ? dim3(std::max(nchunk, ntile), sel.n, 2) : dim3(nchunk, ntile), block(64 * kFieldWaves);
    c->field_part_valid = true;
    c->field_key = key;
    bool fused = false;
    if (c->call.coef_job_valid) {
        const CoefJob &cj = c->call.coef_job;
        fused = c->opt.fuse_field && !skip && sel.n > 0 && !P.polar_ewald && c->graph_mode == GM_DIRECT &&
                (long)grid.x * sel.n * kFieldWaves >= (long)cj.nt * cj.dm.n;
        if (fused) grid.z = 3;
        else if (launch_coef_job(c, bx)) return -1;
    }
    if (P.polar_ewald) {
        if (build_field_kvectors(c)) return -1;
        const int nkc = 8, kchunk = (c->nkf + nkc - 1) / nkc;
        if (c->nkf > 0 && c->graph_mode != GM_UPDATE) {
            hipLaunchKernelGGL(ewald_field_sf_kernel, dim3(c->nkf), dim3(256), 0, c->stream, a, c->d_kvecf, c->d_sf);
            hipLaunchKernelGGL(ewald_field_recip_kernel, dim3(nkc, ntile), dim3(64), 0, c->stream, a, c->d_kvecf, c->d_sf,
                               c->nkf, kchunk, 8.0 * kPI / c->volume, nchunk, c->d_fieldpart);
        }
        fp.wolf_alpha = c->polar_ewald_alpha;
        if (!skip)
            HIPCHK(launch_slot(c, GS_FIELD, static_field_kernel<kFieldEwald>, grid, block, c->stream, a, bx, fp, sel,
                               c->d_fieldpart));
        c->es_slots = nchunk + (c->nkf > 0 ? nkc : 0);
        c->es_stale = true;
        return 0;
    }
    if (mode == kFieldWolfA) {
        const double al = P.polar_wolf_alpha, R = c->cutoff, rR = 1.0 / R;
        fp.cutoffterm = std::erfc(al * R) * rR * rR + 2.0 * al * kOneOverSqrtPi * std::exp(-al * al * R * R) * rR;
    }
#define MPMC_FIELD_DISPATCH(...)                                                       \
    do switch (mode) {                                                                 \
        case kFieldBare: { constexpr int kF = kFieldBare; __VA_ARGS__; break; }        \
        case kFieldWolf0: { constexpr int kF = kFieldWolf0; __VA_ARGS__; break; }      \
        default: { constexpr int kF = kFieldWolfA; __VA_ARGS__; break; }               \
    } while (0)
    if (fused) {
        const CoefJob &cj = c->call.coef_job;
        c->call.coef_job_valid = false;
        MPMC_FIELD_DISPATCH(MPMC_THOLE_DISPATCH(c, hipLaunchKernelGGL((field_coef_kernel<kF, kM>), grid, block, 0, c->stream, a, bx,
                                                                      fp, sel, c->d_fieldpart, cj)));
        HIPCHK(hipGetLastError());
        if (c->call.coef_job_fork) hipEventRecord(c->ev_fork, c->stream);
    } else if (!skip) {
        MPMC_FIELD_DISPATCH(HIPCHK(launch_slot(c, GS_FIELD, static_field_kernel<kF>, grid, block, c->stream, a, bx, fp, sel,
                                               c->d_fieldpart)));
    }
#undef MPMC_FIELD_DISPATCH
    c->es_slots = nchunk;
    c->es_stale = true;
    return 0;
}

static int apply_deferred_moves(mpmc_hip_ctx *c) {
    if (!c->call.moves_deferred) return 0;
    c->call.moves_deferred = false;
    c->call.side_carry = false;
    if (flush_moves(c)) return -1;
    if (c->opt.overlap) hipEventRecord(c->ev_fork, c->stream);
    return 0;
}

static bool collect_dirty_slots(mpmc_hip_ctx *c, const SweepView &v, DirtyList &dl, int &nd) {
    nd = 0;
    for (int atom : c->dirty_atoms) {
        const int slot = v.slot_of_atom[atom];
        if (slot < 0) continue;
        bool seen = false;
        for (int k = 0; k < nd; ++k) seen |= (c->h_dirty[k] == slot);
        if (seen) continue;
        if (nd == kMaxDirty) return false;
        c->h_dirty[nd++] = slot;
    }
    for (int k = 0; k < kMaxDirty; ++k) dl.slot[k] = (k < nd) ? c->h_dirty[k] : 0;
    return true;
}

static int print_inv_stamps(hipStream_t st, const unsigned long long *istamps, size_t nwg, int waves, const GsBuild &gb,
                            int nsingle, bool full) {
    std::vector<unsigned long long> h(nwg * 4);
    HIPCHK(hipStreamSynchronize(st));
    HIPCHK(hipMemcpy(h.data(), istamps, h.size() * sizeof(unsigned long long), hipMemcpyDeviceToHost));
    unsigned long long t0 = ~0ull, t3 = 0;
    double ph[3] = {0, 0, 0}, phmax[3] = {0, 0, 0}, start_max = 0;
    int live = 0;
    for (size_t g = 0; g < nwg; ++g) {
        if (!h[4 * g + 3]) continue;
        t0 = std::min(t0, h[4 * g]);
    }
    for (size_t g = 0; g < nwg; ++g) {
        if (!h[4 * g + 3]) continue;
        ++live;
        t3 = std::max(t3, h[4 * g + 3]);
        start_max = std::max(start_max, (double)(h[4 * g] - t0) * 0.01);
        for (int k = 0; k < 3; ++k) {
            const double d = (double)(h[4 * g + k + 1] - h[4 * g + k]) * 0.01;
            ph[k] += d;
            phmax[k] = std::max(phmax[k], d);
        }
    }
    fprintf(stderr, "INV_STAMPS waves %d, %d live workgroups of %zu (lists %d %d %d, full %d): span %.2f us, last start +%.2f us; "
                    "mean (max) us: loads %.2f (%.2f), expansion %.2f (%.2f), substitution %.2f (%.2f)\n",
            waves, live, nwg, gb.inv.n, gb.own.n, nsingle, full ? 1 : 0, (double)(t3 - t0) * 0.01, start_max, ph[0] / std::max(live, 1),
            phmax[0], ph[1] / std::max(live, 1), phmax[1], ph[2] / std::max(live, 1), phmax[2]);
    return 0;
}

static int maintain_chain_data(mpmc_hip_ctx *c, SweepView &v, const DevBox &bx, hipStream_t st, int nt, bool coef_updated,
// ... 37 lines not shown
                HIPCHK(hipMemsetAsync(c->d_istamps, 0, nwg * 4 * sizeof(unsigned long long), st));
                istamps = c->d_istamps;
            }
        }
#define MPMC_LAUNCH_INVERSE(O, W)                                                                                          \
    hipLaunchKernelGGL((gs_block_inverse_kernel<O, W>), gi, bi, kInverseLds, bst, v.C, v.ntld, v.px, v.py, v.pz, v.palpha, bx, \
                       gb, istamps)
        if (c->box_ortho) {
            if (waves == 4) MPMC_LAUNCH_INVERSE(1, 4);
            else if (waves == 8) MPMC_LAUNCH_INVERSE(1, 8);
            else MPMC_LAUNCH_INVERSE(1, 16);
        } else {
            if (waves == 4) MPMC_LAUNCH_INVERSE(0, 4);
            else if (waves == 8) MPMC_LAUNCH_INVERSE(0, 8);
            else MPMC_LAUNCH_INVERSE(0, 16);
        }
#undef MPMC_LAUNCH_INVERSE
        if (bst != st) {
            HIPCHK(hipEventRecord(c->ev_bjoin, bst));
            c->call.build_join_pending = true;
        }
        if (istamps) {
            --c->opt.inv_stamps;
            if (print_inv_stamps(st, istamps, nwg, waves, gb, nsingle, full)) return -1;
        }
    }
    v.M_epoch = v.C_epoch;
    v.M_call = c->energy_calls;
    return 0;
}

static void hand_over_coef_job(mpmc_hip_ctx *c, const SweepView &v, const DevAtoms &pa, const TholeParams &tp,
                               const DirtyMoves &dm, int nt) {
    CoefJob &cj = c->call.coef_job;
    cj.pa = pa;
    cj.tp = tp;
    cj.dm = dm;
    cj.nt = nt;
    cj.ntld = v.ntld;
    cj.C = v.C;
    cj.m = c->pending;
    cj.gx = c->d_x;
    cj.gy = c->d_y;
    cj.gz = c->d_z;
    cj.slot_of_atom = (const int *)v.d_slot;
    cj.px = v.px;
    cj.py = v.py;
    cj.pz = v.pz;
    c->call.coef_job_valid = true;
    if (c->call.side_carry) c->call.side_moves = c->pending;
    c->pending.n = 0;
    c->call.moves_deferred = false;
    c->call.coef_job_fork = c->opt.overlap && !c->call.side_carry && c->call.side_apply.n == 0;
}

static int setup_view(mpmc_hip_ctx *c, SweepView &v, const DevAtoms &a, const DevBox &bx, bool incremental,
                      bool want_coef, bool want_matrix, bool want_chain = false, hipStream_t side = nullptr) {
    const hipStream_t st = side ? side : c->stream;
    bool fuse_moves = false;
    if (c->call.moves_deferred && &v == &c->view[0]) {
        fuse_moves = !side && incremental && v.pos_valid && want_coef && v.C_valid && v.rebuild_from < 0 && !c->all_dirty &&
                     c->opt.incremental;
        if (!fuse_moves && apply_deferred_moves(c)) return -1;
    }
    if (!(incremental && v.pos_valid)) {
        const dim3 g((v.cap + 255) / 256), b(256);
        hipLaunchKernelGGL(gather_atoms_kernel, g, b, 0, st, v.nv, v.cap, v.d_idx, a, v.px, v.py, v.pz,
                           v.palpha, v.pflags);
        v.pos_valid = incremental && (&v == &c->view[0]);
    }
    DevAtoms pa = a;
    pa.x = v.px;
    pa.y = v.py;
    pa.z = v.pz;
    pa.alpha = v.palpha;
    pa.flags = v.pflags;
    pa.n = v.nv;
    pa.npad = v.nvpad;
    const TholeParams tp = thole_params(c, v.d_idx);
    ScopedTimer t(c, T_AMAT, st);
    DirtyList dl;
    int nd = 0;
    const bool can_update = incremental && !c->all_dirty && c->opt.incremental && collect_dirty_slots(c, v, dl, nd);
    const int nt = std::max(1, (v.nv + kCoefTile - 1) / kCoefTile);
    bool coef_updated = false;
    int tail = -1;
    if (v.rebuild_from >= 0) {
        if (want_coef && want_chain && can_update && v.C_valid && v.rebuild_from < nt && nt - v.rebuild_from <= kMaxBlockList - 16)
            tail = v.rebuild_from;
        else
            v.C_valid = false;
        v.rebuild_from = -1;
    }
    if (want_coef) {
        if (ensure_view_coef(c, v, nt, st)) return -1;
        if (can_update && v.C_valid) {
            if (tail >= 0)
                MPMC_THOLE_DISPATCH(c, hipLaunchKernelGGL((build_coef_kernel<kM>), dim3(nt, nt), dim3(64 * kCoefWaves), 0, st, pa,
                                                          bx, tp, v.ntld, v.C, tail));
            if (nd > 0 && side)
                MPMC_THOLE_DISPATCH(c, hipLaunchKernelGGL((update_coef_kernel<kM>), dim3(nt, nd), dim3(64), 0, st, pa, bx, tp, dl,
                                                          v.ntld, v.C));
            else if (nd > 0 && fuse_moves && nd <= kMaxDirtyMoves) {
                DirtyMoves dm;
                dm.n = nd;
                for (int k = 0; k < kMaxDirtyMoves; ++k) {
                    dm.slot[k] = (k < nd) ? dl.slot[k] : 0;
                    dm.x[k] = dm.y[k] = dm.z[k] = 0.0;
                }
                bool all_found = true;
                for (int k = 0; k < nd; ++k) {
                    const int atom = v.h_idx[dl.slot[k]];
                    bool found = false;
                    for (int e = 0; e < c->pending.n; ++e) {
                        if (c->pending.idx[e] == atom) {
                            dm.x[k] = c->pending.x[e];
                            dm.y[k] = c->pending.y[e];
                            dm.z[k] = c->pending.z[e];
                            found = true;
                        }
                    }
                    all_found &= found;
                }
                if (all_found) {
                    hand_over_coef_job(c, v, pa, tp, dm, nt);
                    if (want_chain && launch_coef_job(c, bx)) return -1;
                } else {
                    if (apply_deferred_moves(c)) return -1;
                    MPMC_THOLE_DISPATCH(c, HIPCHK(launch_slot(c, GS_COEF, update_coef_kernel<kM>, dim3(nt, nd), dim3(64), c->stream,
                                                              pa, bx, tp, dl, v.ntld, v.C)));
                }
            } else if (nd > 0) {
                if (c->call.moves_deferred && &v == &c->view[0] && apply_deferred_moves(c)) return -1;
                MPMC_THOLE_DISPATCH(c, HIPCHK(launch_slot(c, GS_COEF, update_coef_kernel<kM>, dim3(nt, nd), dim3(64), c->stream, pa,
                                                          bx, tp, dl, v.ntld, v.C)));
            }
            if (c->call.moves_deferred && &v == &c->view[0] && apply_deferred_moves(c)) return -1;
            coef_updated = true;
        } else {
            if (c->call.moves_deferred && &v == &c->view[0] && apply_deferred_moves(c)) return -1;
            MPMC_THOLE_DISPATCH(c, hipLaunchKernelGGL((build_coef_kernel<kM>), dim3(nt, nt), dim3(64 * kCoefWaves), 0, st, pa, bx,
                                                      tp, v.ntld, v.C, 0));
            v.C_valid = true;
            ++v.C_epoch;
        }
    } else {
        v.C_valid = false;
    }
    if (want_chain && want_coef && maintain_chain_data(c, v, bx, st, nt, coef_updated, tail, dl, nd)) return -1;
    if (want_matrix) {
        if (ensure_view_matrix(v)) return -1;
        if (can_update && v.A_valid) {
            if (nd > 0)
                MPMC_THOLE_DISPATCH(c, hipLaunchKernelGGL((update_amatrix_kernel<kM>), dim3(v.nvpad / 128, nd), dim3(64), 0, st, pa,
                                                          bx, tp, dl, v.A, 3 * v.nvpad));
        } else {
            MPMC_THOLE_DISPATCH(c, hipLaunchKernelGGL((build_amatrix_kernel<kM>), dim3(v.nvpad / 128, v.nvpad / kARows), dim3(64), 0,
// ... 62 lines not shown
        if (ensure_sym_scratch(v)) return -1;
        {
            ScopedTimer t(c, timer_class);
            const dim3 g(nvpad / kSymChunkAtoms, nvpad / kSymRowAtoms);
            const int rev = (c->opt.sym_mode & 1) ? (c->sweep_parity++ & 1) : 0;
            if (c->opt.sym_mode & 2)
                hipLaunchKernelGGL(symv_kernel<1>, g, dim3(64), 0, c->stream, v.A, lda, nvpad, mu_in, v.Srow, v.Zcol, rev,
                                   v.nv);
            else
                hipLaunchKernelGGL(symv_kernel<0>, g, dim3(64), 0, c->stream, v.A, lda, nvpad, mu_in, v.Srow, v.Zcol, rev,
                                   v.nv);
        }
        ScopedTimer t2(c, T_OTHER);
        hipLaunchKernelGGL(symv_finish_kernel<MODE>, dim3(nvpad / 64), dim3(1024), 0, c->stream, nvpad, v.Srow, v.Zcol,
                           v.palpha, v.pflags, mu_in, v.es, v.efind, out, v.rrms, c->d_errmax, sp);
    } else {
        ScopedTimer t(c, timer_class);
        hipLaunchKernelGGL(sweep_kernel<MODE>, dim3(nvpad), dim3(64), 0, c->stream, v.A, lda, nvpad, v.palpha,
                           v.pflags, mu_in, v.es, v.efind, out, v.rrms, c->d_errmax, sp);
    }
    return 0;
}

static bool defer_last_sweep(const mpmc_hip_ctx *c, const SweepView &v) {
    const mpmc_hip_params &P = c->par;
    if (!c->opt.pair_coef || !v.C_valid) return false;
    if (P.polar_zodid || P.polar_gs || P.polar_gs_ranked || P.polar_palmo || P.polar_sor || P.polar_esor || P.polar_rrms)
        return false;
    if (P.polar_precision != 0.0 || P.polar_gamma != 1.0 || P.polar_max_iter < 2) return false;
    const int nt = std::max(1, (v.nv + kCoefTile - 1) / kCoefTile);
    return nt * (nt + 1) / 2 + nt > c->num_cus;
}

static int complete_pending_sweep(mpmc_hip_ctx *c) {
    if (c->psweep.sweeps.empty()) return 0;
    PendingSweep p;
    std::swap(p, c->psweep);
    HIPCHK(hipSetDevice(c->device));
    for (const PendingSweep::One &s : p.sweeps)
        if (launch_sweep<kSweepJacobi>(c, *p.view, p.bx, s.mu_in, s.mu_out, s.sp, T_SWEEP)) return -1;
    return 0;
}

static void (*chain_kernel_of(int ortho))(GsChain) { return ortho ? gs_chain_kernel<1> : gs_chain_kernel<0>; }

static bool gs_uses_chain(const mpmc_hip_ctx *c) { return c->opt.pair_coef != 0 && c->opt.persistent_gs != 0; }

struct GsFinishArgs {
    double w_new, w_old;
    int want_rrms, err_slot;
    double *mu_out;
};
static int launch_gs_sweep(mpmc_hip_ctx *c, SweepView &v, const DevAtoms &a, const DevBox &bx, const double *mu_old,
                           const GsFinishArgs *fin = nullptr, bool *finished = nullptr) {
    if (finished) *finished = false;
    const int nvpad = v.nvpad, lda = 3 * nvpad;
    (void)a;
    ++c->call.gs_sweeps;
    if (gs_uses_chain(c) && v.C_valid) {
        const int nt = std::max(1, (v.nv + kCoefTile - 1) / kCoefTile);
        if (ensure_coef_scratch(v, nt)) return -1;
        const bool fold_upper = c->opt.gs_fold_upper && fin && c->opt.gs_fold_finish && !c->opt.gs_ablate;
        {
            ScopedTimer tu(c, T_OTHER);
            const dim3 g(nt * (nt + 1) / 2), b(64 * kCoefWaves);
            const int rev = c->opt.sweep_alternate ? (c->sweep_parity++ & 1) : 0;
            if (c->box_ortho)
// ... 567 lines not shown
```

mpmc_amd/csrc/step_plan.h:

```cpp
#pragma once

#include <algorithm>
#include <cmath>
#include <cstring>
#include <utility>
#include <vector>

#include "step_pods.h"

namespace mpmc {

static inline int round_up(int v, int m) { return (v + m - 1) / m * m; }

struct ChunkPlan {
    int nchunk, chunk;
};
static inline ChunkPlan chunk_plan(int npad, int target) {
    const int ntile = npad / 64;
    int nchunk = std::max(1, std::min(ntile, target / ntile));
    const int chunk = round_up((npad + nchunk - 1) / nchunk, 64);
    nchunk = (npad + chunk - 1) / chunk;
    return {nchunk, chunk};
}

static inline bool blocks_of(const std::vector<int> &atoms, DirtyBlocks &out) {
    memset(&out, 0, sizeof(out));
    for (int atom : atoms) {
        const int b = atom / 64;
        bool seen = false;
        for (int k = 0; k < out.n; ++k) seen |= (out.blk[k] == b);
        if (seen) continue;
        if (out.n == kMaxDirtyBlocks) {
            memset(&out, 0, sizeof(out));
            return false;
        }
        out.blk[out.n++] = b;
    }
    return true;
}

static inline bool place_molecule(const std::vector<std::pair<int, int>> &holes, int n, int max_atoms, int count, int &first,
                                  int &hole) {
    first = hole = -1;
    for (int h = (int)holes.size() - 1; h >= 0; --h)
        if (holes[h].second == count) {
            hole = h;
            first = holes[h].first;
            return true;
        }
    if (n + count > max_atoms) return false;
    first = n;
    return true;
}
static inline int count_new_view_slots(const std::vector<int> &slot_of_atom, bool gs_mode, int first, int count,
                                       const double *polarizability) {
    int new_view = 0;
    for (int i = 0; i < count; ++i) {
        const bool had = !gs_mode && first + i < (int)slot_of_atom.size() && slot_of_atom[first + i] >= 0;
        if (polarizability[i] != 0.0 && !had) ++new_view;
    }
    return new_view;
}

static inline void mixing_weights(bool sor, bool esor, double gamma, int k, double &w_new, double &w_old) {
    w_new = 1.0;
    w_old = 0.0;
    if (sor) {
        w_new = gamma;
        w_old = 1.0 - gamma;
// ... 110 lines not shown
```

mpmc_amd/csrc/step_pods.h:

```cpp
#pragma once

namespace mpmc {

constexpr int kMaxDirtyBlocks = 16;
struct DirtyBlocks {
    int n;
    int blk[kMaxDirtyBlocks];
};

struct SweepParams {
    double w_new;
    double w_old;
    int want_rrms;
    int want_err;
    int err_slot;
    int skip_sums;
    int energy_mode = 0;
};
constexpr int kEnergyStoreSums = 1;
constexpr int kEnergyMid = 2;
constexpr int kEnergyPrevSums = 4;

constexpr int kGsMaxLag = 4;

constexpr int kMaxBlockList = 48;
struct BlockList {
    int n;
    int blk[kMaxBlockList];
};

struct GsBuild {
    BlockList inv;
    BlockList own;
    BlockList nb[kGsMaxLag];
    double *Minv;
    double *Lnb[kGsMaxLag];
    int nlag;
    int nb_all;
};

// ... 2 lines not shown
```

mpmc_amd/engine.py:

```python
import ctypes as C
import os

import numpy as np

_HERE = os.path.dirname(os.path.abspath(__file__))
LIB_PATH = os.path.join(_HERE, "csrc", "libmpmc_hip.so")

EXPORTS = [
    "mpmc_hip_last_error", "mpmc_hip_abi_version", "mpmc_hip_device_count", "mpmc_hip_create",
    "mpmc_hip_destroy", "mpmc_hip_set_option", "mpmc_hip_default_params", "mpmc_hip_set_params", "mpmc_hip_set_box",
    "mpmc_hip_scale_box",
    "mpmc_hip_upload", "mpmc_hip_set_dispersion", "mpmc_hip_set_axilrod_teller", "mpmc_hip_get_three_body_energy",
    "mpmc_hip_set_rd_crystal", "mpmc_hip_set_rd_form", "mpmc_hip_set_vdw", "mpmc_hip_get_vdw_energy", "mpmc_hip_get_vdw_terms",
    "mpmc_hip_set_autoreject", "mpmc_hip_get_close_contacts",
    "mpmc_hip_set_cavity_grid", "mpmc_hip_cavity_bin", "mpmc_hip_cavity_update", "mpmc_hip_cavity_point",
    "mpmc_hip_download_cavity_grid",
    "mpmc_hip_set_exact_polar", "mpmc_hip_get_polarizability_tensor", "mpmc_hip_set_thole_model",
    "mpmc_hip_update_atoms", "mpmc_hip_insert_molecule", "mpmc_hip_remove_molecule", "mpmc_hip_edit_molecules",
    "mpmc_hip_slot_count", "mpmc_hip_set_sweep_order", "mpmc_hip_energy", "mpmc_hip_energy_begin", "mpmc_hip_energy_end",
    "mpmc_hip_download_dipoles",
    "mpmc_hip_download_amatrix", "mpmc_hip_download_ranking", "mpmc_hip_get_timings",
    "mpmc_hip_comm_unique_id", "mpmc_hip_comm_create", "mpmc_hip_comm_size", "mpmc_hip_comm_rank",
    "mpmc_hip_allreduce_observables", "mpmc_hip_allreduce_observables_begin", "mpmc_hip_allreduce_observables_end",
    "mpmc_hip_gather_observables", "mpmc_hip_comm_destroy",
]


class Params(C.Structure):
    _fields_ = [
        ("temperature", C.c_double),
        ("rd_only", C.c_int),
        ("rd_lrc", C.c_int),
        ("feynman_hibbs", C.c_int),
        ("feynman_hibbs_order", C.c_int),
        ("ewald_alpha_set", C.c_int),
        ("ewald_alpha", C.c_double),
        ("ewald_kmax", C.c_int),
        ("polarization", C.c_int),
        ("polar_damp", C.c_double),
        ("polar_max_iter", C.c_int),
        ("polar_precision", C.c_double),
        ("polar_gamma", C.c_double),
        ("polar_gs", C.c_int),
        ("polar_gs_ranked", C.c_int),
        ("polar_sor", C.c_int),
        ("polar_esor", C.c_int),
        ("polar_palmo", C.c_int),
        ("polar_rrms", C.c_int),
        ("polar_zodid", C.c_int),
        ("polar_wolf", C.c_int),
        ("polar_wolf_alpha", C.c_double),
        ("polar_ewald", C.c_int),
# ... 13 lines not shown
        ("es_recip", C.c_double),
        ("es_self", C.c_double),
        ("dipole_rrms", C.c_double),
        ("volume", C.c_double),
        ("cutoff", C.c_double),
        ("ewald_alpha", C.c_double),
        ("polar_ewald_alpha", C.c_double),
        ("polar_iterations", C.c_int),
        ("iter_success", C.c_int),
        ("n_atoms", C.c_int),
        ("status", C.c_int),
    ]


class Timings(C.Structure):
    _fields_ = [
        ("pair_ms", C.c_float),
        ("recip_ms", C.c_float),
        ("field_ms", C.c_float),
        ("amatrix_ms", C.c_float),
        ("sweep_ms", C.c_float),
        ("palmo_ms", C.c_float),
        ("other_ms", C.c_float),
        ("total_ms", C.c_float),
        ("sweep_count", C.c_int),
        ("amatrix_count", C.c_int),
        ("graph_steps", C.c_int),
        ("event_pair_ms", C.c_float),
        ("event_pair_count", C.c_int),
        ("spec_rank_redos", C.c_int),
        ("resident_calls", C.c_int),
        ("resident_fallbacks", C.c_int),
        ("pending_sweeps", C.c_int),
    ]


class DispParams(C.Structure):
    _fields_ = [
        ("disp_expansion", C.c_int),
        ("damp_dispersion", C.c_int),
        ("extrapolate_disp_coeffs", C.c_int),
        ("schmidt_mixing", C.c_int),
    ]


class RdFormParams(C.Structure):
    _fields_ = [
        ("form", C.c_int),
        ("mixing", C.c_int),
    ]


class TholeModel(C.Structure):
    _fields_ = [
        ("damp_type", C.c_int),
        ("wolf_full", C.c_int),
    ]


class Molecule(C.Structure):
    _fields_ = [("count", C.c_int), ("frozen", C.c_int)] + [
        (k, C.c_void_p) for k in ("x", "y", "z", "charge", "polarizability", "epsilon", "sigma", "mass",
                                  "c6", "c8", "c10", "c9")]


THOLE_DAMPINGS = {"off": 0, "none": 0, "linear": 1, "exponential": 2}
# ... 38 lines not shown
    lib.mpmc_hip_default_params.restype = None
    lib.mpmc_hip_set_params.argtypes = [vp, C.POINTER(Params)]
    lib.mpmc_hip_set_box.argtypes = [vp, dp, C.c_double]
    lib.mpmc_hip_scale_box.argtypes = [vp, dp, C.c_double, C.c_int, vp]
    lib.mpmc_hip_upload.argtypes = [vp, C.c_int] + [vp] * 10
    lib.mpmc_hip_set_dispersion.argtypes = [vp, C.POINTER(DispParams), C.c_int, vp, vp, vp]
    lib.mpmc_hip_set_axilrod_teller.argtypes = [vp, C.c_int, C.c_int, vp]
    lib.mpmc_hip_get_three_body_energy.argtypes = [vp, dp]
    lib.mpmc_hip_set_rd_crystal.argtypes = [vp, C.c_int]
    lib.mpmc_hip_set_rd_form.argtypes = [vp, C.POINTER(RdFormParams)]
    lib.mpmc_hip_set_vdw.argtypes = [vp, C.c_int, C.c_int, vp, vp]
    lib.mpmc_hip_get_vdw_energy.argtypes = [vp, dp]
    lib.mpmc_hip_get_vdw_terms.argtypes = [vp, dp]
    lib.mpmc_hip_set_exact_polar.argtypes = [vp, C.c_int]
    lib.mpmc_hip_get_polarizability_tensor.argtypes = [vp, dp]
    lib.mpmc_hip_set_thole_model.argtypes = [vp, C.POINTER(TholeModel)]
    lib.mpmc_hip_set_autoreject.argtypes = [vp, C.c_double]
    lib.mpmc_hip_get_close_contacts.argtypes = [vp, C.POINTER(C.c_longlong)]
    ip = C.POINTER(C.c_int)
    lib.mpmc_hip_set_cavity_grid.argtypes = [vp, C.c_int, C.c_double]
    lib.mpmc_hip_cavity_bin.argtypes = [vp, C.c_int, vp, vp, vp]
    lib.mpmc_hip_cavity_update.argtypes = [vp, C.c_int, vp, C.c_int, vp, C.c_int, vp, ip, ip]
    lib.mpmc_hip_cavity_point.argtypes = [vp, C.c_int, ip, dp]
    lib.mpmc_hip_download_cavity_grid.argtypes = [vp, vp, vp]
    lib.mpmc_hip_update_atoms.argtypes = [vp, C.c_int, C.c_int, vp, vp, vp]
    lib.mpmc_hip_insert_molecule.argtypes = [vp, C.c_int, vp, vp, vp, vp, vp, vp, vp, vp, C.c_int, C.POINTER(C.c_int)]
    lib.mpmc_hip_remove_molecule.argtypes = [vp, C.c_int, C.c_int]
    lib.mpmc_hip_edit_molecules.argtypes = [vp, C.c_int, vp, vp, C.c_int, C.POINTER(Molecule), vp]
    lib.mpmc_hip_slot_count.argtypes = [vp]
    lib.mpmc_hip_set_sweep_order.argtypes = [vp, C.c_int, vp]
    lib.mpmc_hip_energy.argtypes = [vp, C.POINTER(Result)]
    lib.mpmc_hip_energy_begin.argtypes = [vp]
    lib.mpmc_hip_energy_end.argtypes = [vp, C.POINTER(Result)]
    lib.mpmc_hip_download_dipoles.argtypes = [vp, vp, vp, vp, vp]
    lib.mpmc_hip_download_amatrix.argtypes = [vp, vp]
    lib.mpmc_hip_download_ranking.argtypes = [vp, vp, vp]
    lib.mpmc_hip_get_timings.argtypes = [vp, C.POINTER(Timings)]
    lib.mpmc_hip_comm_unique_id.argtypes = [vp]
    lib.mpmc_hip_comm_create.argtypes = [C.POINTER(vp), vp, C.c_int, C.c_int, vp]
    lib.mpmc_hip_allreduce_observables.argtypes = [vp, vp, C.c_int]
    lib.mpmc_hip_allreduce_observables_begin.argtypes = [vp, vp, C.c_int]
    lib.mpmc_hip_allreduce_observables_end.argtypes = [vp, vp]
    lib.mpmc_hip_gather_observables.argtypes = [vp, vp, C.c_int, vp]
    lib.mpmc_hip_comm_size.argtypes = [vp]
    lib.mpmc_hip_comm_rank.argtypes = [vp]
    lib.mpmc_hip_comm_destroy.argtypes = [vp]
    lib.mpmc_hip_comm_destroy.restype = None
    _lib = lib
    return lib


class EngineError(RuntimeError):
    pass


def _chk(rc):
    if rc != 0:
        raise EngineError(load().mpmc_hip_last_error().decode())


def make_params(**kw):
    p = Params()
    load().mpmc_hip_default_params(C.byref(p))
    for k, v in kw.items():
        if k in NOT_PARAMS:
            continue
# ... 241 lines not shown
                setattr(m, name, keep[-1].ctypes.data)
            for field, key in (("charge", "charge"), ("polarizability", "alpha"), ("epsilon", "epsilon"),
                               ("sigma", "sigma"), ("mass", "mass"), ("c6", "c6"), ("c8", "c8"), ("c10", "c10"), ("c9", "c9")):
                if d.get(key) is None:
                    continue
                a = np.ascontiguousarray(d[key], dtype=np.float64)
                if a.shape != (pos.shape[0],):
                    raise ValueError("edit_molecules: %s must have one entry per atom of the molecule" % key)
                keep.append(a)
                setattr(m, field, a.ctypes.data)
        first = np.full(max(1, len(insert)), -1, dtype=np.int32)
        rc = self.lib.mpmc_hip_edit_molecules(self.ctx, len(remove), rf.ctypes.data if remove else None,
                                              rk.ctypes.data if remove else None, len(insert),
                                              mols if len(insert) else None, first.ctypes.data if len(insert) else None)
        if rc < 0:
            _chk(rc)
        if rc > 0:
            return None
        self.n = int(self.lib.mpmc_hip_slot_count(self.ctx))
        return [int(f) for f in first[:len(insert)]]

    def set_sweep_order(self, slots):
        a = np.ascontiguousarray(slots, dtype=np.int32)
        _chk(self.lib.mpmc_hip_set_sweep_order(self.ctx, len(a), a.ctypes.data))

    def energy(self):
        r = Result()
        _chk(self.lib.mpmc_hip_energy(self.ctx, C.byref(r)))
        return {f: getattr(r, f) for f, _ in Result._fields_}

    def energy_begin(self):
        _chk(self.lib.mpmc_hip_energy_begin(self.ctx))

    def energy_end(self):
        r = Result()
        _chk(self.lib.mpmc_hip_energy_end(self.ctx, C.byref(r)))
        return {f: getattr(r, f) for f, _ in Result._fields_}

    def dipoles(self):
        out = {k: np.zeros((self.n, 3)) for k in ("mu", "ef_static", "ef_induced", "ef_induced_change")}
        _chk(self.lib.mpmc_hip_download_dipoles(self.ctx, out["mu"].ctypes.data, out["ef_static"].ctypes.data,
                                                out["ef_induced"].ctypes.data,
                                                out["ef_induced_change"].ctypes.data))
        return out

    def amatrix(self):
        A = np.zeros((3 * self.n, 3 * self.n))
        _chk(self.lib.mpmc_hip_download_amatrix(self.ctx, A.ctypes.data))
        return A

    def ranking(self):
        rank = np.zeros(self.n)
        order = np.zeros(self.n, dtype=np.int32)
        _chk(self.lib.mpmc_hip_download_ranking(self.ctx, rank.ctypes.data, order.ctypes.data))
        return rank, order

    def timings(self):
        t = Timings()
        _chk(self.lib.mpmc_hip_get_timings(self.ctx, C.byref(t)))
        return {f: getattr(t, f) for f, _ in Timings._fields_}
```

mpmc_amd/host.py:

```python
import ctypes as C
import os

import numpy as np

from . import engine

_HERE = os.path.dirname(os.path.abspath(__file__))
LIB_PATH = os.environ.get("MPMC_HOST_LIB") or os.path.join(_HERE, "host", "libmpmc_host.so")
EXE_PATH = os.path.join(_HERE, "host", "mpmc_hip")

_lib = None


def load():
    global _lib
    if _lib is not None:
        return _lib
    if not os.path.exists(LIB_PATH):
        raise RuntimeError("mpmc_amd/host/libmpmc_host.so is not built (run __graft_entry__.build())")
    engine.load()
    lib = C.CDLL(LIB_PATH)
    vp = C.c_void_p
    lib.system_from_arrays.restype = vp
    lib.system_from_arrays.argtypes = [C.c_int] + [vp] * 9
# ... 12 lines not shown
    lib.host_get_dipoles.argtypes = [vp, vp, vp, vp]
    lib.host_natoms.argtypes = [vp]
    lib.host_get_system.argtypes = [vp] * 9
    lib.host_seed.argtypes = [vp, C.c_uint]
    lib.host_mc_steps_multi.argtypes = [C.POINTER(vp), C.c_int, C.c_int]
    lib.host_mc_steps_multi.restype = C.c_int
    lib.host_get_rand.argtypes = [vp]
    lib.host_get_rand.restype = C.c_double
    lib.energy.argtypes = [vp]
    lib.energy.restype = C.c_double
    lib.mc.argtypes = [vp]
    lib.countNatoms.argtypes = [vp]
    lib.translate.argtypes = [vp, vp, vp, C.c_double]
    lib.checkpoint.argtypes = [vp]
    lib.make_move.argtypes = [vp]
    lib.restore.argtypes = [vp]
    lib.walkers_unique_id.argtypes = [vp]
    lib.walkers_init.argtypes = [vp, C.c_int, C.c_int, vp]
    lib.walkers_pool_begin.argtypes = [vp, vp, C.c_int]
    lib.walkers_pool_end.argtypes = [vp, vp, C.c_int]
    lib.walkers_finalize.argtypes = [vp]
    lib.walkers_finalize.restype = None
    lib.host_device_error.argtypes = [vp]
    lib.host_get_basis.argtypes = [vp, vp]
    lib.host_get_basis.restype = None
    lib.host_get_npt.argtypes = [vp, vp]
    lib.host_get_npt.restype = None
    lib.host_set_volume_notes.argtypes = [vp, C.c_int]
    lib.host_set_volume_notes.restype = None
    lib.host_force_volume_move.argtypes = [vp, C.c_double, C.c_int]
    lib.host_force_volume_move.restype = None
    lib.host_init_chain_no_energy.argtypes = [vp]
    lib.host_init_chain_no_energy.restype = None
    lib.host_get_disp_flags.argtypes = [vp, vp]
    lib.host_get_disp_flags.restype = None
    lib.host_get_dispersion.argtypes = [vp, vp, vp, vp]
    lib.host_get_dispersion.restype = None
    lib.host_set_dispersion.argtypes = [vp, vp, vp, vp]
    lib.host_set_dispersion.restype = None
    lib.host_get_at_flags.argtypes = [vp, vp]
    lib.host_get_at_flags.restype = None
    lib.host_get_c9.argtypes = [vp, vp]
    lib.host_get_c9.restype = None
    lib.host_set_c9.argtypes = [vp, vp]
    lib.host_set_c9.restype = None
    lib.host_get_three_body_energy.argtypes = [vp]
    lib.host_get_three_body_energy.restype = C.c_double
    lib.host_get_vdw.argtypes = [vp, vp]
    lib.host_get_vdw.restype = None
    lib.host_get_omega.argtypes = [vp, vp]
    lib.host_get_omega.restype = None
    lib.host_set_omega.argtypes = [vp, vp, vp]
    lib.host_set_omega.restype = None
    lib.host_displace_molecule.argtypes = [vp, C.c_int, vp]
    lib.host_get_rdc_flags.argtypes = [vp, vp]
    lib.host_get_rdc_flags.restype = None
    lib.host_get_rdform_flags.argtypes = [vp, vp]
    lib.host_get_rdform_flags.restype = None
    lib.host_get_thole_flags.argtypes = [vp, vp]
    lib.host_get_thole_flags.restype = None
    lib.host_read_frame.argtypes = [vp, C.c_char_p, C.c_int]
    lib.host_unsupported.argtypes = [vp]
    lib.host_unsupported.restype = C.c_char_p
    lib.host_get_polarizability_tensor.argtypes = [vp, vp]
    lib.host_get_cavity_flags.argtypes = [vp, vp]
    lib.host_get_cavity_flags.restype = None
# ... 139 lines not shown
        self.lib.host_get_cavity_darts(self.ptr, darts.ctypes.data)
        return darts

    def observables(self):
        out = np.zeros(8)
        self.lib.host_get_observables(self.ptr, out.ctypes.data)
        npt = np.zeros(5)
        self.lib.host_get_npt(self.ptr, npt.ctypes.data)
        return dict(energy=out[0], coulombic_energy=out[1], rd_energy=out[2], polarization_energy=out[3], N=out[4],
                    polar_iterations=out[5], accept=int(out[6]), reject=int(out[7]), volume=npt[0], cutoff=npt[1],
                    accept_volume=int(npt[2]), reject_volume=int(npt[3]))

    def basis(self):
        b = np.zeros(9)
        self.lib.host_get_basis(self.ptr, b.ctypes.data)
        return b.reshape(3, 3)

    def next_movetype(self):
        npt = np.zeros(5)
        self.lib.host_get_npt(self.ptr, npt.ctypes.data)
        return ("insert", "remove", "displace", "volume")[int(npt[4])]

    def set_volume_notes(self, on):
        self.lib.host_set_volume_notes(self.ptr, int(bool(on)))

    def force_volume_move(self, new_volume, revert=False):
        self.lib.host_force_volume_move(self.ptr, float(new_volume), int(bool(revert)))

    def sync_counts(self):
        out = (C.c_long * 3)()
        self.lib.host_get_sync_counts(self.ptr, out)
        return dict(full_uploads=int(out[0]), edit_calls=int(out[1]), molecules_edited=int(out[2]))

    def mc_steps(self, nsteps):
        r = self.lib.host_mc_steps(self.ptr, int(nsteps))
        if r < 0:
            raise engine.EngineError(engine.load().mpmc_hip_last_error().decode())
        return r

    def walkers_init(self, nranks, rank, unique_id):
        buf = (C.c_ubyte * 128).from_buffer_copy(bytes(unique_id)) if unique_id is not None else None
        if self.lib.walkers_init(self.ptr, int(nranks), int(rank), buf) != 0:
            raise engine.EngineError("walkers_init: " + engine.load().mpmc_hip_last_error().decode())

    def pool_begin(self, values):
        v = np.ascontiguousarray(values, dtype=np.float64)
        if self.lib.walkers_pool_begin(self.ptr, v.ctypes.data, len(v)) != 0:
            raise engine.EngineError("walkers_pool_begin: " + engine.load().mpmc_hip_last_error().decode())

    def pool_end(self, count):
        out = np.zeros(count)
        if self.lib.walkers_pool_end(self.ptr, out.ctypes.data, count) != 0:
            raise engine.EngineError("walkers_pool_end: " + engine.load().mpmc_hip_last_error().decode())
        return out

    def positions(self):
        pos = np.zeros((self.natoms(), 3))
        self.lib.host_get_positions(self.ptr, pos.ctypes.data)
        return pos

    def natoms(self):
        return int(self.lib.host_natoms(self.ptr))

    def system(self, basis):
        n = self.natoms()
        f = {k: np.zeros(n) for k in ("charge", "alpha", "epsilon", "sigma", "mass")}
# ... 23 lines not shown
```

mpmc_amd/host/energy_hip.c:

```c
#include <math.h>
#include <stdint.h>
#include <stdio.h>
#include <stdlib.h>
#include <string.h>
#include <time.h>

#ifdef MPMC_SHIM_HOST_MIRROR
#include "mpmc_host.h"
#else
#include <structs.h>
#include <function_prototypes.h>
extern int rank, size;
#endif
#include "energy_hip.h"


typedef struct {
    molecule_t *mol;
    atom_t *atoms;
    int slot, natoms, frozen;
} resident_t;

typedef struct {
    molecule_t *mol;
// ... 87 lines not shown
    for (int v = 0; v < st->nvol; v++) free(st->vol_delta[v]);
    free(st->res); free(st->res2); free(st->mols);
    free(st->cav); free(st->cav2); free(st->cav_raw); free(st->cav_raw2); free(st->cav_wrapped); free(st->cav_wrapped2);
    free(st->cav_darts);
    free(st);
}

void energy_hip_set_device(system_t *system, int device) {
    shim_state *st = state_of(system, 1);
    if (st) st->device = device;
}
mpmc_hip_ctx *energy_hip_context(system_t *system) {
    shim_state *st = state_of(system, 0);
    return st ? st->ctx : NULL;
}
int energy_hip_failed(system_t *system) {
    shim_state *st = state_of(system, 0);
    return st ? st->failed : 0;
}
double energy_hip_last_energy(system_t *system) {
    shim_state *st = state_of(system, 0);
    return st ? st->last_energy : 0.0;
}
void energy_hip_enable_timing(system_t *system, int on) {
    shim_state *st = state_of(system, 1);
    if (!st) return;
    st->timing = on;
    memset(&st->tsum, 0, sizeof(st->tsum));
}
void energy_hip_get_timings(system_t *system, mpmc_hip_timings *out) {
    shim_state *st = state_of(system, 0);
    if (st) *out = st->tsum;
    else memset(out, 0, sizeof(*out));
}

static double g_prof[4];
static long g_prof_calls, g_prof_base;
static double g_prof_t0, g_prof_tlast;
static double now_s(void) { struct timespec t; clock_gettime(CLOCK_MONOTONIC, &t); return t.tv_sec + 1e-9 * t.tv_nsec; }
void energy_hip_profile_report(void) {
    if (getenv("MPMC_HIP_HOST_PROFILE") && g_prof_calls)
    {
        const long nc = g_prof_calls - g_prof_base > 0 ? g_prof_calls - g_prof_base : 1;
        fprintf(stderr, "host energy(): %ld steady-state calls; list work + updates %.1f us, begin %.1f us, bookkeeping %.1f us, "
                        "end %.1f us per call; %.1f us per call between energy() calls (MC logic)\n", nc,
                1e6 * g_prof[0] / nc, 1e6 * g_prof[1] / nc, 1e6 * g_prof[2] / nc, 1e6 * g_prof[3] / nc,
                1e6 * ((g_prof_tlast - g_prof_t0) - (g_prof[0] + g_prof[1] + g_prof[2] + g_prof[3])) / nc);
    }
}

#ifdef MPMC_SHIM_HOST_MIRROR
int countNatoms(system_t *system) {
    int N = 0;
    for (molecule_t *m = system->molecules; m; m = m->next)
        for (atom_t *a = m->atoms; a; a = a->next) N++;
    return N;
}
static void countN(system_t *system) {
    system->observables->N = 0;
    system->observables->spin_ratio = 0;
    for (molecule_t *m = system->molecules; m; m = m->next)
        if (!m->frozen) system->observables->N += 1.0;
}
void update_com(molecule_t *molecules) {
    for (molecule_t *m = molecules; m; m = m->next) {
        for (int i = 0; i < 3; i++) m->com[i] = 0;
// ... 872 lines not shown
            st->ctx = NULL;
            st->cav_ctx = NULL;
        }
        if (!st->ctx) {
            st->capacity = system->natoms + (system->ensemble == ENSEMBLE_UVT ? system->natoms / 2 + 1024 : 0);
            int device = st->device;
            if (device < 0) {
#ifdef MPMC_SHIM_HOST_MIRROR
                device = 0;
#else
                const int ndev = mpmc_hip_device_count();
                device = ndev > 0 ? rank % ndev : 0;
#endif
            }
            if (mpmc_hip_create(&st->ctx, device, st->capacity)) {
                hip_fail("create");
                return device_failed(st);
            }
            st->device = device;
            st->uploaded = 0;
        }
        if (full_upload(st, system)) return device_failed(st);
    }
    const double t1 = now_s();
    if (mpmc_hip_energy_begin(st->ctx)) {
        hip_fail("energy");
        return device_failed(st);
    }
    g_prof[0] += t1 - t0;
    g_prof[1] += now_s() - t1;
    return 0;
}

double energy_hip_end(system_t *system) {
    shim_state *st = state_of(system, 0);
    if (!st || !st->ctx) return NAN;
    const double t2 = now_s();
    update_com(system->molecules);
    countN(system);
    const double t3 = now_s();
    mpmc_hip_result r;
    if (mpmc_hip_energy_end(st->ctx, &r)) {
        hip_fail("energy");
        device_failed(st);
        return NAN;
    }
    const double t4 = now_s();
    g_prof[2] += t3 - t2; g_prof[3] += t4 - t3;
    if (++g_prof_calls == 64) {
        g_prof[0] = g_prof[1] = g_prof[2] = g_prof[3] = 0.0;
        g_prof_t0 = t4;
        g_prof_base = 64;
    }
    g_prof_tlast = t4;
    if (st->timing) {
        mpmc_hip_timings t;
        if (!mpmc_hip_get_timings(st->ctx, &t)) {
            mpmc_hip_timings *s = &st->tsum;
            s->pair_ms += t.pair_ms; s->recip_ms += t.recip_ms; s->field_ms += t.field_ms;
            s->amatrix_ms += t.amatrix_ms; s->sweep_ms += t.sweep_ms; s->palmo_ms += t.palmo_ms;
            s->other_ms += t.other_ms; s->total_ms += t.total_ms;
            s->sweep_count += t.sweep_count; s->amatrix_count += t.amatrix_count;
            s->event_pair_ms += t.event_pair_ms; s->event_pair_count += t.event_pair_count;
            s->spec_rank_redos = t.spec_rank_redos;
            s->resident_calls = t.resident_calls;
            s->resident_fallbacks = t.resident_fallbacks;
// ... 209 lines not shown
```

mpmc_amd/host/energy_hip.h:

```cpp
#ifndef ENERGY_HIP_H
#define ENERGY_HIP_H

#include <mpmc_hip.h>

#ifdef __cplusplus
extern "C" {
#endif

double energy_hip(system_t *system);
int energy_hip_begin(system_t *system);
double energy_hip_end(system_t *system);
int energy_hip_failed(system_t *system);
const char *energy_hip_unsupported(const system_t *system);

void energy_hip_note_moved(system_t *system, molecule_t *now, molecule_t *was);
void energy_hip_note_list_changed(system_t *system);
void energy_hip_note_volume_change(system_t *system, const double *delta_per_molecule);
void energy_hip_set_volume_notes(system_t *system, int on);

void energy_hip_sync_counts(system_t *system, long out[3]);
double energy_hip_effective_c9(int midzuno_kihara_approx, double alpha, double c6, double c9);

int energy_hip_download_dipoles(system_t *system);
int energy_hip_corrtime(system_t *system);

int energy_hip_polarizability_tensor(system_t *system, double tensor[9], int print);

int energy_hip_cavity_update(system_t *system);
int energy_hip_cavity_point(system_t *system, int index, double com[3]);
int energy_hip_cavity_darts(system_t *system, const double **darts, int *hits);

void energy_hip_cleanup(system_t *system);

void energy_hip_set_device(system_t *system, int device);
mpmc_hip_ctx *energy_hip_context(system_t *system);
double energy_hip_last_energy(system_t *system);
void energy_hip_enable_timing(system_t *system, int on);
void energy_hip_get_timings(system_t *system, mpmc_hip_timings *out);
void energy_hip_profile_report(void);

int walkers_unique_id(unsigned char id[128]);
int walkers_init(system_t *system, int nranks, int rank, const unsigned char id[128]);
int walkers_init_from_env(system_t *system);
int walkers_gather(system_t *system, const void *snd_strct, int msgsize, void *rcv_strct);
int walkers_pool_begin(system_t *system, const double *values, int count);
int walkers_pool_end(system_t *system, double *values, int count);
// ... 7 lines not shown
```

mpmc_amd/host/mc.c:

```c
#include <math.h>
#include <stdlib.h>
#include <string.h>

#include "mpmc_host.h"

void seed_rng(system_t *system, unsigned int seed) {
    unsigned int *mt = system->rng_mt;
    int mti;
    mt[0] = seed;
    for (mti = 1; mti < 624; mti++) mt[mti] = 1812433253u * (mt[mti - 1] ^ (mt[mti - 1] >> 30)) + (unsigned int)mti;
    system->rng_mti = mti;
}

static unsigned int mt_next(system_t *system) {
    unsigned int *mt = system->rng_mt;
    if (system->rng_mti >= 624) {
        for (int k = 0; k < 624; k++) {
            unsigned int y = (mt[k] & 0x80000000u) | (mt[(k + 1) % 624] & 0x7fffffffu);
            mt[k] = mt[(k + 397) % 624] ^ (y >> 1) ^ ((y & 1u) ? 0x9908b0dfu : 0u);
        }
        system->rng_mti = 0;
    }
    unsigned int y = mt[system->rng_mti++];
    y ^= (y >> 11);
// ... 339 lines not shown
        case MOVETYPE_REMOVE:
            energy_hip_note_list_changed(system);
            system->movable_valid = 0;
            if (!cp->head)
                system->molecules = cp->molecule_backup;
            else
                cp->head->next = cp->molecule_backup;
            cp->molecule_backup->next = cp->tail;
            cp->molecule_backup = NULL;
            break;
        case MOVETYPE_VOLUME:
            revert_volume_change(system);
            break;
        default:
            if (cp->molecule_altered) {
                if (!cp->head)
                    system->molecules = cp->molecule_backup;
                else
                    cp->head->next = cp->molecule_backup;
                cp->molecule_backup->next = cp->tail;
                energy_hip_note_moved(system, cp->molecule_backup, cp->molecule_altered);
                if (system->movable_valid) {
                    const int k = cp->altered_index;
                    system->movable[k] = cp->molecule_backup;
                    if (k + 1 < system->nmovable && system->movable_prev[k + 1] == cp->molecule_altered)
                        system->movable_prev[k + 1] = cp->molecule_backup;
                }
                free_molecule(system, cp->molecule_altered);
                cp->molecule_altered = NULL;
                cp->molecule_backup = NULL;
            }
    }
    checkpoint(system);
}

void boltzmann_factor(system_t *system, double initial_energy, double final_energy) {
    const double delta_energy = final_energy - initial_energy;
    double bf = exp(-delta_energy / system->temperature);
    if (system->ensemble == ENSEMBLE_UVT) {
        const double fugacity = system->fugacity;
        if (system->cavity_bias && system->checkpoint->biased_move) {
            if (system->checkpoint->movetype == MOVETYPE_INSERT)
                bf = (system->cavity_volume * system->avg_nodestats->cavity_bias_probability * fugacity * ATM2REDUCED /
                      (system->temperature * system->observables->N)) *
                     exp(-delta_energy / system->temperature);
            else if (system->checkpoint->movetype == MOVETYPE_REMOVE)
                bf = (system->temperature * (system->observables->N + 1.0)) /
                     (system->cavity_volume * system->avg_nodestats->cavity_bias_probability * fugacity * ATM2REDUCED) *
                     exp(-delta_energy / system->temperature);
        } else if (system->checkpoint->movetype == MOVETYPE_INSERT)
            bf = system->pbc->volume * fugacity * ATM2REDUCED / (system->temperature * (double)(system->observables->N)) *
                 exp(-delta_energy / system->temperature);
        else if (system->checkpoint->movetype == MOVETYPE_REMOVE)
            bf = system->temperature * ((double)(system->observables->N) + 1.0) /
                 (system->pbc->volume * fugacity * ATM2REDUCED) * exp(-delta_energy / system->temperature);
    } else if (system->ensemble == ENSEMBLE_NPT && system->checkpoint->movetype == MOVETYPE_VOLUME) {
        const double v_old = system->checkpoint->observables->volume;
        const double v_new = system->observables->volume;
        bf = exp(-(delta_energy + system->pressure * ATM2REDUCED * (v_new - v_old) -
                   (system->observables->N + 1) * system->temperature * log(v_new / v_old)) /
                 system->temperature);
    }
    system->nodestats->boltzmann_factor = bf;
}

void write_observables(FILE *fp, system_t *system, observables_t *o, double core_temp) {
// ... 51 lines not shown
    char linebuf[MAXLINE];
    system->observables->volume = system->pbc->volume;
    system->observables->temperature = 0;

    if (system->cavity_bias) energy_hip_cavity_update(system);

    system->step = 0;
    initial_energy = energy(system);
    if (energy_hip_failed(system)) return -1;
    const int size = getenv("MPMC_HIP_NRANKS") ? atoi(getenv("MPMC_HIP_NRANKS")) : 1;
    const int rank = getenv("MPMC_HIP_RANK") ? atoi(getenv("MPMC_HIP_RANK")) : 0;
    if (walkers_init_from_env(system) < 0) return -1;
    walker_record_t snd, *rcv = calloc(size > 0 ? size : 1, sizeof(walker_record_t));
    if (!rcv) return -1;
    if (!isfinite(initial_energy)) initial_energy = system->observables->energy = MAXVALUE;

    if (!rank && system->energy_output[0] && !system->fp_energy) {
        system->fp_energy = fopen(system->energy_output, "w");
        if (!system->fp_energy) {
            error("MC: could not open files\n");
            return -1;
        }
        fprintf(system->fp_energy,
                "#step #energy #coulombic #rd #polar #vdw #kinetic #kin_temp #N #spin_ratio #volume #core_temp\n");
    }
    if (!rank) update_averages(system, system->observables, system->nodestats->polarization_iterations);
    if (system->fp_energy) write_observables(system->fp_energy, system, system->observables, system->temperature);

    checkpoint(system);

    for (system->step = 1; system->step <= system->numsteps; (system->step)++) {
        initial_energy = system->observables->energy;
        make_move(system);
        final_energy = energy(system);
        if (energy_hip_failed(system)) {
            error("MC: the device engine failed, stopping the chain\n");
            free(rcv);
            return -1;
        }
        if (!isfinite(final_energy)) {
            system->observables->energy = MAXVALUE;
            system->nodestats->boltzmann_factor = 0;
        } else
            boltzmann_factor(system, initial_energy, final_energy);

        const int volume_move = system->checkpoint->movetype == MOVETYPE_VOLUME;
        if ((get_rand(system) < system->nodestats->boltzmann_factor) && (system->iter_success == 0)) {
            checkpoint(system);
            ++system->nodestats->accept;
            if (volume_move)
                ++system->nodestats->accept_volume;
            else
                ++system->nodestats->accept_displace;
        } else {
            system->iter_success = 0;
            restore(system);
            ++system->nodestats->reject;
            if (volume_move)
                ++system->nodestats->reject_volume;
            else
                ++system->nodestats->reject_displace;
        }
        system->nodestats->acceptance_rate =
            (double)system->nodestats->accept / (double)(system->nodestats->accept + system->nodestats->reject);
        update_nodestats(system->nodestats, system->avg_nodestats);

        if (!(system->step % system->corrtime)) {
// ... 26 lines not shown
```

mpmc_amd/host/mpmc_host.h:

```cpp
#ifndef MPMC_HOST_H
#define MPMC_HOST_H

#include <stdio.h>

#include <mpmc_hip.h>

#ifdef __cplusplus
extern "C" {
#endif

#define MAXLINE 512
#define MAXVALUE 1.0e40
#define E2REDUCED 408.7816
#define ATM2REDUCED 0.0073389366

enum { ENSEMBLE_UVT, ENSEMBLE_NVT, ENSEMBLE_SURF, ENSEMBLE_SURF_FIT, ENSEMBLE_NVE, ENSEMBLE_TE, ENSEMBLE_NPT,
       ENSEMBLE_REPLAY };
enum { MOVETYPE_INSERT, MOVETYPE_REMOVE, MOVETYPE_DISPLACE, MOVETYPE_VOLUME };
enum { DAMPING_OFF, DAMPING_LINEAR, DAMPING_EXPONENTIAL };

typedef struct _atom {
    int id, bond_id;
    char atomtype[MAXLINE];
    int frozen;
// ... 102 lines not shown
    nodestats_t *nodestats;
    avg_nodestats_t *avg_nodestats;
    avg_observables_t *avg_observables;
    checkpoint_t *checkpoint;
    double last_volume;
    struct _molecule **movable, **movable_prev;
    int nmovable, movable_cap, movable_valid;
    FILE *fp_energy;
} system_t;

system_t *setup_system(char *input_file);
system_t *read_config(char *input_file);
int do_command(system_t *system, char **token);
molecule_t *read_molecules(FILE *fp, system_t *system);
void pbc(system_t *system);
int check_cavity_bias(system_t *system);
system_t *system_from_arrays(int n, const double *pos, const double *charge, const double *polarizability,
                             const double *epsilon, const double *sigma, const double *mass, const int *molecule,
                             const int *frozen, const double basis[9]);
void free_system(system_t *system);

double energy(system_t *system);
int countNatoms(system_t *system);
void update_com(molecule_t *molecules);

int mc(system_t *system);
int replay_trajectory(system_t *system);
int read_frame(FILE *fp, system_t *system);
void write_observables(FILE *fp, system_t *system, observables_t *o, double core_temp);
void checkpoint(system_t *system);
void restore(system_t *system);
void make_move(system_t *system);
void boltzmann_factor(system_t *system, double initial_energy, double final_energy);
void update_nodestats(nodestats_t *nodestats, avg_nodestats_t *avg_nodestats);
void clear_avg_nodestats(system_t *system);
void update_root_nodestats(system_t *system, avg_nodestats_t *avg_nodestats, avg_observables_t *avg_observables);
double get_rand(system_t *system);
void seed_rng(system_t *system, unsigned int seed);
molecule_t *copy_molecule(system_t *system, molecule_t *src);
void free_molecule(system_t *system, molecule_t *molecule);
void translate(system_t *system, molecule_t *molecule, pbc_t *pbc, double scale);
void rotate(system_t *system, molecule_t *molecule, pbc_t *pbc, double scale);
void volume_change(system_t *system);
void volume_change_to(system_t *system, double new_volume);
void revert_volume_change(system_t *system);
int wrapall(molecule_t *molecules, pbc_t *pbc);

void output(const char *msg);
void error(const char *msg);
int write_molecules(system_t *system, const char *filename);

#ifdef __cplusplus
}
#endif

#include "energy_hip.h"
#endif
```

Measured before the change: 14010 MC steps/s.

## Speculatively prefetch next MC displacement's head computation during current energy evaluation

```diff
diff --git a/include/mpmc_hip.h b/include/mpmc_hip.h
--- a/include/mpmc_hip.h
+++ b/include/mpmc_hip.h
@@ -74,6 +74,7 @@
     int resident_calls;
     int resident_fallbacks;
     int pending_sweeps;
+    int prefetch_issued, prefetch_used, prefetch_overwritten, prefetch_cancelled;
 } mpmc_hip_timings;
 
 const char *mpmc_hip_last_error(void);
@@ -180,6 +181,8 @@
 int mpmc_hip_energy_begin(mpmc_hip_ctx *ctx);
 int mpmc_hip_energy_end(mpmc_hip_ctx *ctx, mpmc_hip_result *out);
 
+int mpmc_hip_prefetch_atoms(mpmc_hip_ctx *ctx, int first, int count, const double *x, const double *y, const double *z);
+
 int mpmc_hip_download_dipoles(mpmc_hip_ctx *ctx, double *mu, double *ef_static, double *ef_induced,
                               double *ef_induced_change);
 
diff --git a/mpmc_amd/csrc/device_common.h b/mpmc_amd/csrc/device_common.h
--- a/mpmc_amd/csrc/device_common.h
+++ b/mpmc_amd/csrc/device_common.h
@@ -38,12 +38,6 @@
     int tie_guard;
 };
 
-constexpr int kMaxMoves = 32;
-struct MoveList {
-    int n;
-    int idx[kMaxMoves];
-    double x[kMaxMoves], y[kMaxMoves], z[kMaxMoves];
-};
 struct MoveTargets {
     double *x, *y, *z;
     const int *slot_of_atom;
diff --git a/mpmc_amd/csrc/engine.hip b/mpmc_amd/csrc/engine.hip
--- a/mpmc_amd/csrc/engine.hip
+++ b/mpmc_amd/csrc/engine.hip
@@ -272,6 +272,12 @@
     int graph = 0;
 };
 
+struct PrefetchedHead {
+    bool outstanding = false;
+    MoveList fwd{}, old{};
+    unsigned long long config_rev = 0;
+};
+
 struct CallState {
     bool do_polar = false;
     bool gs_mode = false;
@@ -292,6 +298,8 @@
     bool coef_job_valid = false;
     bool coef_job_fork = false;
     CoefJob coef_job;
+    bool head_fused = false;
+    bool head_prefetched = false;
     bool build_join_pending = false;
     bool rank_on_side = false;
     int gs_sweeps = 0;
@@ -478,6 +486,13 @@
     bool force_multi_launch = false;
     bool res_attr_set = false;
     unsigned long long resident_calls = 0, resident_fallbacks = 0;
+    PrefetchedHead pf;
+    int prefetch_head = 0;
+    std::vector<double> mir_x, mir_y, mir_z;
+    bool mirror_valid = false;
+    unsigned long long pf_issued = 0, pf_used = 0, pf_overwritten = 0, pf_cancelled = 0, pf_skipped = 0;
+    unsigned long long pf_polls = 0, pf_poll_timeouts = 0;
+    double pf_poll_s = 0.0, pf_poll_max_s = 0.0;
     int graph_mode = 0;
     StepGraph sg;
     int eligible_streak = 0;
@@ -587,6 +602,7 @@
     } while (0)
 
 static int complete_pending_sweep(mpmc_hip_ctx *c);
+static int cancel_prefetch(mpmc_hip_ctx *c);
 template <int NRHS>
 static int exact_substitute(mpmc_hip_ctx *c, int nv, int nvpad, const double *es);
 static void drop_polar_result(mpmc_hip_ctx *c) {
@@ -754,6 +770,10 @@
     }
     if (complete_pending_sweep(c)) return -1;
     ++c->config_rev;
+    if (!strcmp(name, "prefetch_head")) {
+        c->prefetch_head = value;
+        return 0;
+    }
     for (const OptionRow &o : kOptions) {
         if (strcmp(name, o.name)) continue;
         if (o.hook) return o.hook(c, value);
@@ -907,6 +927,15 @@
     if (getenv("MPMC_HIP_HOST_PROFILE") && c->graph_launches)
         fprintf(stderr, "MPMC_HIP graph steps: node updates %.1f us, launch %.1f us per step\n",
                 1e6 * c->graph_update_s / c->graph_launches, 1e6 * c->graph_launch_s / c->graph_launches);
+    if (c->pf.outstanding) {
+        c->pf.outstanding = false;
+        ++c->pf_cancelled;
+    }
+    if (getenv("MPMC_HIP_HOST_PROFILE") && (c->pf_issued || c->pf_skipped))
+        fprintf(stderr, "MPMC_HIP head prefetch: issued %llu used %llu overwritten %llu cancelled %llu skipped %llu; wait for the side "
+                        "record: %llu polls, mean %.1f us, max %.1f us, %llu gave up\n",
+                c->pf_issued, c->pf_used, c->pf_overwritten, c->pf_cancelled, c->pf_skipped, c->pf_polls,
+                c->pf_polls ? 1e6 * c->pf_poll_s / c->pf_polls : 0.0, 1e6 * c->pf_poll_max_s, c->pf_poll_timeouts);
     hipSetDevice(c->device);
     hipStreamSynchronize(c->stream);
     hipStreamSynchronize(c->stream2);
@@ -1039,6 +1068,10 @@
     if (!x || !y || !z || !charge || !polarizability || !epsilon || !sigma || !mass || !molecule || !frozen)
         return fail("MPMC_HIP: upload: null array");
     HIPCHK(hipSetDevice(c->device));
+    if (c->pf.outstanding) {
+        c->pf.outstanding = false;
+        ++c->pf_cancelled;
+    }
     drop_polar_result(c);
     const int npad = round_up(n, 128);
     const int nall = c->max_npad;
@@ -1080,6 +1113,10 @@
     HIPCHK(hipStreamSynchronize(c->stream));
     c->coord_max = 0.0;
     note_coords(c, x, y, z, n);
+    c->mir_x.assign(x, x + n);
+    c->mir_y.assign(y, y + n);
+    c->mir_z.assign(z, z + n);
+    c->mirror_valid = true;
     c->n = n;
     c->npad = npad;
     c->n_valid = n;
@@ -1158,6 +1195,7 @@
     if (per_atom_setter_refused(c, "set_dispersion")) return -1;
     if (n != c->n) return fail("MPMC_HIP: set_dispersion: %d coefficients for the %d atoms of the upload", n, c->n);
     HIPCHK(hipSetDevice(c->device));
+    if (cancel_prefetch(c)) return -1;
     if (flush_moves(c)) return -1;
     c->disp.valid = c->disp_lrc.valid = false;
     lj_kernels_switched(c);
@@ -1200,6 +1238,7 @@
     if (!c) return fail("MPMC_HIP: set_axilrod_teller: null context");
     if (per_atom_setter_refused(c, "set_axilrod_teller")) return -1;
     HIPCHK(hipSetDevice(c->device));
+    if (cancel_prefetch(c)) return -1;
     if (!enable) {
         if (flush_moves(c)) return -1;
         c->at_on = false;
@@ -1237,6 +1276,7 @@
 extern "C" int mpmc_hip_set_rd_crystal(mpmc_hip_ctx *c, int order) {
     if (!c) return fail("MPMC_HIP: set_rd_crystal: null context");
     if (c->in_flight) return fail("MPMC_HIP: set_rd_crystal between energy_begin() and energy_end()");
+    if (cancel_prefetch(c)) return -1;
     if (order < 0 || order > kRdcMaxOrder)
         return fail("MPMC_HIP: set_rd_crystal: rd_crystal_order %d outside 1 .. %d (0 = off)", order, kRdcMaxOrder);
     if (order == c->rdc_order) return 0;
@@ -1364,6 +1404,7 @@
     if (!c) return fail("MPMC_HIP: set_vdw: null context");
     if (per_atom_setter_refused(c, "set_vdw")) return -1;
     HIPCHK(hipSetDevice(c->device));
+    if (cancel_prefetch(c)) return -1;
     if (!enable) {
         c->vdw_iso.clear();
         if (!c->vdw_on) return 0;
@@ -1448,6 +1489,7 @@
 extern "C" int mpmc_hip_set_autoreject(mpmc_hip_ctx *c, double scale) {
     if (!c) return fail("MPMC_HIP: set_autoreject: null context");
     if (c->in_flight) return fail("MPMC_HIP: set_autoreject between energy_begin() and energy_end()");
+    if (cancel_prefetch(c)) return -1;
     if (!(scale >= 0.0) || !std::isfinite(scale)) return fail("MPMC_HIP: set_autoreject: scale %g (0 = off)", scale);
     if (scale == c->autoreject_scale) return 0;
     HIPCHK(hipSetDevice(c->device));
@@ -1502,6 +1544,11 @@
     if (!x || !y || !z) return fail("MPMC_HIP: update_atoms: null array");
     HIPCHK(hipSetDevice(c->device));
     note_coords(c, x, y, z, count);
+    if (c->mirror_valid) {
+        std::copy(x, x + count, c->mir_x.begin() + first);
+        std::copy(y, y + count, c->mir_y.begin() + first);
+        std::copy(z, z + count, c->mir_z.begin() + first);
+    }
     const size_t b = count * sizeof(double);
     bool queued = false;
     if (count <= kMaxMoves) {
@@ -1597,6 +1644,7 @@
         c->stage_used = 0;
     }
     if (apply_box(c, basis, pbc_cutoff)) return -1;
+    c->mirror_valid = false;
     double *s = c->h_stage + c->stage_used;
     memcpy(s, delta, need * sizeof(double));
     c->stage_used += need;
@@ -1684,6 +1732,7 @@
     drop_polar_result(c);
     if (flush_moves(c)) return -1;
     c->main_writes = true;
+    c->mirror_valid = false;
     hipLaunchKernelGGL(apply_edits_kernel, dim3(1), dim3(64), 0, c->stream, ed, t);
     HIPCHK(hipGetLastError());
     return 0;
@@ -1720,6 +1769,7 @@
 extern "C" int mpmc_hip_remove_molecule(mpmc_hip_ctx *c, int first, int count) {
     if (!c || !c->have_atoms) return fail("MPMC_HIP: remove_molecule: no configuration uploaded");
     if (c->in_flight) return fail("MPMC_HIP: remove_molecule between energy_begin() and energy_end()");
+    if (cancel_prefetch(c)) return -1;
     if (first < 0 || count <= 0 || first + count > c->n)
         return fail("MPMC_HIP: remove_molecule: range [%d, %d) outside [0, %d)", first, first + count, c->n);
     for (int i = 0; i < count; ++i)
@@ -1759,6 +1809,7 @@
                                         const double *sigma, const double *mass, int frozen, int *first_slot) {
     if (!c || !c->have_atoms) return fail("MPMC_HIP: insert_molecule: no configuration uploaded");
     if (c->in_flight) return fail("MPMC_HIP: insert_molecule between energy_begin() and energy_end()");
+    if (cancel_prefetch(c)) return -1;
     if (count <= 0 || !x || !y || !z || !charge || !polarizability || !epsilon || !sigma || !mass || !first_slot)
         return fail("MPMC_HIP: insert_molecule: bad arguments");
     if (count > kMaxEdit || !edits_supported(c)) return 1;
@@ -1848,6 +1899,7 @@
                                        int ninsert, const mpmc_hip_molecule *insert, int *insert_first_slot) {
     if (!c || !c->have_atoms) return fail("MPMC_HIP: edit_molecules: no configuration uploaded");
     if (c->in_flight) return fail("MPMC_HIP: edit_molecules between energy_begin() and energy_end()");
+    if (cancel_prefetch(c)) return -1;
     if (nremove < 0 || ninsert < 0 || (nremove > 0 && (!remove_first_slot || !remove_count)) ||
         (ninsert > 0 && (!insert || !insert_first_slot)))
         return fail("MPMC_HIP: edit_molecules: bad arguments");
@@ -1925,6 +1977,7 @@
 extern "C" int mpmc_hip_set_sweep_order(mpmc_hip_ctx *c, int count, const int *slots) {
     if (!c || !c->have_atoms) return fail("MPMC_HIP: set_sweep_order: no configuration uploaded");
     if (c->in_flight) return fail("MPMC_HIP: set_sweep_order between energy_begin() and energy_end()");
+    if (cancel_prefetch(c)) return -1;
     if (!gs_order_mode(c)) return 0;
     SweepView &v0 = c->view[0];
     if (count < 0 || count > v0.cap || (count > 0 && !slots)) return fail("MPMC_HIP: set_sweep_order: bad arguments");
@@ -2110,6 +2163,7 @@
 }
 
 static int ensure_static_field(mpmc_hip_ctx *c) {
+    if (cancel_prefetch(c)) return -1;
     if (!c->es_stale) return 0;
     hipLaunchKernelGGL(field_reduce_kernel, dim3(c->npad / 64), dim3(64 * kFieldGroups), 0, c->stream, c->d_fieldpart,
                        c->es_slots, c->npad, c->d_es);
@@ -2913,6 +2967,39 @@
     return 0;
 }
 
+static int resolve_prefetch(mpmc_hip_ctx *c, bool &used) {
+    used = false;
+    PrefetchedHead &pf = c->pf;
+    if (!pf.outstanding) return 0;
+    if (c->prefetch_head && !c->main_writes && !c->staged_copies &&
+        prefetch_is_used(c->pending, pf.fwd, c->dirty_atoms, c->all_dirty, c->config_rev, pf.config_rev)) {
+        pf.outstanding = false;
+        used = true;
+        return 0;
+    }
+    int missing = 0;
+    for (int e = 0; e < pf.fwd.n; ++e) missing += move_index(c->pending, pf.fwd.idx[e]) < 0;
+    if (c->pending.n + missing > kMaxMoves) return cancel_prefetch(c);
+    pf.outstanding = false;
+    ++c->pf_overwritten;
+    if (!prefetch_is_covered(c->pending, pf.fwd)) c->main_writes = true;
+    for (int e = 0; e < pf.old.n; ++e) {
+        const int atom = pf.old.idx[e];
+        if (move_index(c->pending, atom) < 0) {
+            MoveList &m = c->pending;
+            m.idx[m.n] = atom;
+            m.x[m.n] = pf.old.x[e];
+            m.y[m.n] = pf.old.y[e];
+            m.z[m.n] = pf.old.z[e];
+            ++m.n;
+        }
+        if (!c->all_dirty && std::find(c->dirty_atoms.begin(), c->dirty_atoms.end(), atom) == c->dirty_atoms.end())
+            c->dirty_atoms.push_back(atom);
+    }
+    if ((int)c->dirty_atoms.size() > 4 * kMaxDirty) c->all_dirty = true;
+    return 0;
+}
+
 extern "C" int mpmc_hip_energy_begin(mpmc_hip_ctx *c) {
     if (!c) return fail("MPMC_HIP: energy: null argument");
     if (c->in_flight) return fail("MPMC_HIP: energy_begin: the previous evaluation has not been collected");
@@ -2936,7 +3023,10 @@
     }
     timespec ts0, ts1;
     clock_gettime(CLOCK_MONOTONIC, &ts0);
+    bool head_prefetched = false;
+    if (resolve_prefetch(c, head_prefetched)) return -1;
     begin_call(c);
+    c->call.head_prefetched = head_prefetched;
     bool issued = false;
     if (graph_eligible(c)) {
         if (c->sg.valid && c->sg.rev == c->config_rev) {
@@ -2983,6 +3073,10 @@
         c->eligible_streak = 0;
     }
     if (!issued && enqueue_direct(c)) return -1;
+    if (c->call.head_prefetched) {
+        c->call.head_prefetched = false;
+        ++c->pf_overwritten;
+    }
     c->staged_copies = false;
     c->main_writes = false;
     clock_gettime(CLOCK_MONOTONIC, &ts1);
@@ -2993,6 +3087,80 @@
     return 0;
 }
 
+static constexpr double kPrefetchPollSeconds = 100e-6;
+
+extern "C" int mpmc_hip_prefetch_atoms(mpmc_hip_ctx *c, int first, int count, const double *x, const double *y,
+                                       const double *z) {
+    if (!c || !x || !y || !z) return fail("MPMC_HIP: prefetch_atoms: null argument");
+    if (!c->in_flight) return fail("MPMC_HIP: prefetch_atoms outside energy_begin() / energy_end()");
+    if (first < 0 || count <= 0 || first + count > c->n)
+        return fail("MPMC_HIP: prefetch_atoms: range [%d, %d) outside [0, %d)", first, first + count, c->n);
+    const CallState &k = c->call;
+    const mpmc_hip_params &P = c->par;
+    const SweepView &v0 = c->view[0];
+    bool ok = c->prefetch_head && !c->pf.outstanding && count <= kMaxMoves && c->mirror_valid && k.do_polar &&
+              k.plain_launches && k.split && k.polar_first && k.head_fused && !k.timed && !k.gs_mode && !k.exact &&
+              !P.polar_zodid && !P.polar_ewald && P.polar_precision == 0.0 && !c->opt.graph && c->pending.n == 0 &&
+              c->dirty_atoms.empty() && !c->all_dirty && !c->main_writes && v0.C_valid && v0.pos_valid &&
+              c->field_part_valid && c->edited == false;
+    double vmax = 0.0;
+    for (int i = 0; ok && i < count; ++i) {
+        const double v = std::max(std::fabs(x[i]), std::max(std::fabs(y[i]), std::fabs(z[i])));
+        if (!(v <= vmax)) vmax = (v == v) ? v : INFINITY;
+    }
+    if (ok && (vmax > kScreen32MaxCoord) && !(c->coord_max > kScreen32MaxCoord)) ok = false;
+    if (!ok) {
+        ++c->pf_skipped;
+        return 0;
+    }
+    {
+        const double want = (double)c->energy_calls;
+        volatile double *seq = c->h_res2 + R_COUNT;
+        timespec t0, t1;
+        clock_gettime(CLOCK_MONOTONIC, &t0);
+        double waited = 0.0;
+        bool seen = (*seq == want);
+        while (!seen && waited < kPrefetchPollSeconds) {
+            for (int s = 0; s < 32 && !seen; ++s) {
+                __builtin_ia32_pause();
+                seen = (*seq == want);
+            }
+            clock_gettime(CLOCK_MONOTONIC, &t1);
+            waited = (t1.tv_sec - t0.tv_sec) + 1e-9 * (t1.tv_nsec - t0.tv_nsec);
+        }
+        ++c->pf_polls;
+        c->pf_poll_s += waited;
+        c->pf_poll_max_s = std::max(c->pf_poll_max_s, waited);
+        if (!seen) {
+            ++c->pf_poll_timeouts;
+            ++c->pf_skipped;
+            return 0;
+        }
+    }
+    HIPCHK(hipSetDevice(c->device));
+    PrefetchedHead &pf = c->pf;
+    pf.fwd.n = pf.old.n = count;
+    for (int i = 0; i < count; ++i) {
+        pf.fwd.idx[i] = pf.old.idx[i] = first + i;
+        pf.fwd.x[i] = x[i];
+        pf.fwd.y[i] = y[i];
+        pf.fwd.z[i] = z[i];
+        pf.old.x[i] = c->mir_x[first + i];
+        pf.old.y[i] = c->mir_y[first + i];
+        pf.old.z[i] = c->mir_z[first + i];
+    }
+    bool done = false;
+    if (enqueue_head_for_moves(c, pf.fwd, done)) return -1;
+    if (!done) {
+        ++c->pf_skipped;
+        return 0;
+    }
+    pf.outstanding = true;
+    pf.config_rev = c->config_rev;
+    ++c->pf_issued;
+    return 1;
+}
+
 static int wait_sequence(volatile double *seq, double want, hipStream_t stream) {
     for (unsigned long long spins = 0; spins < 2000000000ull; ++spins) {
         if (*seq == want) return 0;
@@ -3010,6 +3178,7 @@
 }
 
 static int repeat_call(mpmc_hip_ctx *c, bool &flag) {
+    if (cancel_prefetch(c)) return -1;
     flag = true;
     begin_call(c);
     const int rc = enqueue_direct(c);
@@ -3135,6 +3304,7 @@
     if (!c || !c->have_atoms || !c->have_box || !A) return fail("MPMC_HIP: download_amatrix: no configuration");
     HIPCHK(hipSetDevice(c->device));
     const size_t n3 = 3 * (size_t)c->n, lda = 3 * (size_t)c->npad;
+    if (cancel_prefetch(c)) return -1;
     if (flush_moves(c)) return -1;
     DevBuf<double> dA;
     HIPCHK(dA.alloc(lda * lda));
@@ -3380,6 +3550,10 @@
     t->resident_calls = (int)c->resident_calls;
     t->resident_fallbacks = (int)c->resident_fallbacks;
     t->pending_sweeps = (int)c->psweep.sweeps.size();
+    t->prefetch_issued = (int)c->pf_issued;
+    t->prefetch_used = (int)c->pf_used;
+    t->prefetch_overwritten = (int)c->pf_overwritten;
+    t->prefetch_cancelled = (int)c->pf_cancelled;
     if (!c->timed) return 0;
     HIPCHK(hipSetDevice(c->device));
     float acc[T_NCLASS] = {0};
diff --git a/mpmc_amd/csrc/engine_polar.inc b/mpmc_amd/csrc/engine_polar.inc
--- a/mpmc_amd/csrc/engine_polar.inc
+++ b/mpmc_amd/csrc/engine_polar.inc
@@ -11,31 +11,64 @@
     return 0;
 }
 
+struct FieldPlan {
+    FieldParams fp;
+    int mode, key, nchunk, ntile;
+};
+static FieldPlan field_plan(const mpmc_hip_ctx *c) {
+    const mpmc_hip_params &P = c->par;
+    FieldPlan f;
+    f.fp.wolf_alpha = P.polar_wolf_alpha;
+    f.fp.cutoffterm = 0.0;
+    f.ntile = c->npad / 64;
+    const ChunkPlan cp = chunk_plan(c->npad, 4096);
+    f.nchunk = cp.nchunk;
+    f.fp.chunk = cp.chunk;
+    const bool wolf = P.polar_wolf || c->thole_wolf_full;
+    f.mode = P.polar_ewald ? kFieldEwald : (!wolf ? kFieldBare : (P.polar_wolf_alpha == 0.0 ? kFieldWolf0 : kFieldWolfA));
+    f.key = f.mode * 1000003 + cp.chunk;
+    if (f.mode == kFieldWolfA) {
+        const double al = P.polar_wolf_alpha, R = c->cutoff, rR = 1.0 / R;
+        f.fp.cutoffterm = std::erfc(al * R) * rR * rR + 2.0 * al * kOneOverSqrtPi * std::exp(-al * al * R * R) * rR;
+    }
+    return f;
+}
+static dim3 field_grid(const FieldPlan &f, const DirtyBlocks &sel) {
+    return (sel.n > 0) ? dim3(std::max(f.nchunk, f.ntile), sel.n, 2) : dim3(f.nchunk, f.ntile);
+}
+static bool coef_job_fits(const dim3 &grid, const DirtyBlocks &sel, const CoefJob &cj) {
+    return sel.n > 0 && (long)grid.x * sel.n * kFieldWaves >= (long)cj.nt * cj.dm.n;
+}
+#define MPMC_FIELD_DISPATCH(...)                                                       \
+    do switch (mode) {                                                                 \
+        case kFieldBare: { constexpr int kF = kFieldBare; __VA_ARGS__; break; }        \
+        case kFieldWolf0: { constexpr int kF = kFieldWolf0; __VA_ARGS__; break; }      \
+        default: { constexpr int kF = kFieldWolfA; __VA_ARGS__; break; }               \
+    } while (0)
+#define MPMC_LAUNCH_HEAD(c, grid, a, bx, fp, sel, cj)                                                                         \
+    do {                                                                                                                      \
+        MPMC_FIELD_DISPATCH(MPMC_THOLE_DISPATCH(c, hipLaunchKernelGGL((field_coef_kernel<kF, kM>), grid, dim3(64 * kFieldWaves), 0, \
+                                                                      (c)->stream, a, bx, fp, sel, (c)->d_fieldpart, cj)));   \
+        HIPCHK(hipGetLastError());                                                                                            \
+    } while (0)
+
 static int launch_field(mpmc_hip_ctx *c, const DevAtoms &a, const DevBox &bx) {
     const mpmc_hip_params &P = c->par;
     ScopedTimer t(c, T_FIELD);
-    FieldParams fp;
-    fp.wolf_alpha = P.polar_wolf_alpha;
-    fp.cutoffterm = 0.0;
-    const int ntile = c->npad / 64;
-    const ChunkPlan cp = chunk_plan(c->npad, 4096);
-    const int nchunk = cp.nchunk, chunk = cp.chunk;
-    fp.chunk = chunk;
-    const bool wolf = P.polar_wolf || c->thole_wolf_full;
-    const int mode = P.polar_ewald ? kFieldEwald : (!wolf ? kFieldBare : (P.polar_wolf_alpha == 0.0 ? kFieldWolf0 : kFieldWolfA));
-    const int key = mode * 1000003 + chunk;
+    const FieldPlan plan = field_plan(c);
+    FieldParams fp = plan.fp;
+    const int ntile = plan.ntile, nchunk = plan.nchunk, mode = plan.mode, key = plan.key;
     DirtyBlocks sel = c->call.dirty_blocks;
     const bool resident = c->field_part_valid && c->field_key == key;
     if (!resident) sel.n = 0;
     const bool skip = resident && sel.n == 0 && c->dirty_atoms.empty();
-    dim3 grid = (sel.n > 0) ? dim3(std::max(nchunk, ntile), sel.n, 2) : dim3(nchunk, ntile), block(64 * kFieldWaves);
+    dim3 grid = field_grid(plan, sel), block(64 * kFieldWaves);
     c->field_part_valid = true;
     c->field_key = key;
     bool fused = false;
     if (c->call.coef_job_valid) {
         const CoefJob &cj = c->call.coef_job;
-        fused = c->opt.fuse_field && !skip && sel.n > 0 && !P.polar_ewald && c->graph_mode == GM_DIRECT &&
-                (long)grid.x * sel.n * kFieldWaves >= (long)cj.nt * cj.dm.n;
+        fused = c->opt.fuse_field && !skip && !P.polar_ewald && c->graph_mode == GM_DIRECT && coef_job_fits(grid, sel, cj);
         if (fused) grid.z = 3;
         else if (launch_coef_job(c, bx)) return -1;
     }
@@ -55,28 +88,21 @@
         c->es_stale = true;
         return 0;
     }
-    if (mode == kFieldWolfA) {
-        const double al = P.polar_wolf_alpha, R = c->cutoff, rR = 1.0 / R;
-        fp.cutoffterm = std::erfc(al * R) * rR * rR + 2.0 * al * kOneOverSqrtPi * std::exp(-al * al * R * R) * rR;
-    }
-#define MPMC_FIELD_DISPATCH(...)                                                       \
-    do switch (mode) {                                                                 \
-        case kFieldBare: { constexpr int kF = kFieldBare; __VA_ARGS__; break; }        \
-        case kFieldWolf0: { constexpr int kF = kFieldWolf0; __VA_ARGS__; break; }      \
-        default: { constexpr int kF = kFieldWolfA; __VA_ARGS__; break; }               \
-    } while (0)
     if (fused) {
         const CoefJob &cj = c->call.coef_job;
         c->call.coef_job_valid = false;
-        MPMC_FIELD_DISPATCH(MPMC_THOLE_DISPATCH(c, hipLaunchKernelGGL((field_coef_kernel<kF, kM>), grid, block, 0, c->stream, a, bx,
-                                                                      fp, sel, c->d_fieldpart, cj)));
-        HIPCHK(hipGetLastError());
+        c->call.head_fused = true;
+        if (c->call.head_prefetched) {
+            c->call.head_prefetched = false;
+            ++c->pf_used;
+        } else {
+            MPMC_LAUNCH_HEAD(c, grid, a, bx, fp, sel, cj);
+        }
         if (c->call.coef_job_fork) hipEventRecord(c->ev_fork, c->stream);
     } else if (!skip) {
         MPMC_FIELD_DISPATCH(HIPCHK(launch_slot(c, GS_FIELD, static_field_kernel<kF>, grid, block, c->stream, a, bx, fp, sel,
                                                c->d_fieldpart)));
     }
-#undef MPMC_FIELD_DISPATCH
     c->es_slots = nchunk;
     c->es_stale = true;
     return 0;
@@ -91,19 +117,77 @@
     return 0;
 }
 
-static bool collect_dirty_slots(mpmc_hip_ctx *c, const SweepView &v, DirtyList &dl, int &nd) {
+static bool slots_of(const SweepView &v, const int *atoms, int natoms, int *slots, int &nd) {
     nd = 0;
-    for (int atom : c->dirty_atoms) {
-        const int slot = v.slot_of_atom[atom];
+    for (int q = 0; q < natoms; ++q) {
+        const int slot = v.slot_of_atom[atoms[q]];
         if (slot < 0) continue;
         bool seen = false;
-        for (int k = 0; k < nd; ++k) seen |= (c->h_dirty[k] == slot);
+        for (int k = 0; k < nd; ++k) seen |= (slots[k] == slot);
         if (seen) continue;
         if (nd == kMaxDirty) return false;
-        c->h_dirty[nd++] = slot;
-    }
+        slots[nd++] = slot;
+    }
+    return true;
+}
+static bool collect_dirty_slots(mpmc_hip_ctx *c, const SweepView &v, DirtyList &dl, int &nd) {
+    if (!slots_of(v, c->dirty_atoms.data(), (int)c->dirty_atoms.size(), c->h_dirty.get(), nd)) return false;
     for (int k = 0; k < kMaxDirty; ++k) dl.slot[k] = (k < nd) ? c->h_dirty[k] : 0;
     return true;
+}
+
+static bool fill_dirty_moves(const SweepView &v, const int *slots, int nd, const MoveList &m, DirtyMoves &dm) {
+    dm.n = nd;
+    for (int k = 0; k < kMaxDirtyMoves; ++k) {
+        dm.slot[k] = (k < nd) ? slots[k] : 0;
+        dm.x[k] = dm.y[k] = dm.z[k] = 0.0;
+    }
+    bool all_found = true;
+    for (int k = 0; k < nd; ++k) {
+        const int atom = v.h_idx[slots[k]];
+        bool found = false;
+        for (int e = 0; e < m.n; ++e) {
+            if (m.idx[e] == atom) {
+                dm.x[k] = m.x[e];
+                dm.y[k] = m.y[e];
+                dm.z[k] = m.z[e];
+                found = true;
+            }
+        }
+        all_found &= found;
+    }
+    return all_found;
+}
+
+static DevAtoms view_atoms(const DevAtoms &a, const SweepView &v) {
+    DevAtoms pa = a;
+    pa.x = v.px;
+    pa.y = v.py;
+    pa.z = v.pz;
+    pa.alpha = v.palpha;
+    pa.flags = v.pflags;
+    pa.n = v.nv;
+    pa.npad = v.nvpad;
+    return pa;
+}
+static int view_tiles(const SweepView &v) { return std::max(1, (v.nv + kCoefTile - 1) / kCoefTile); }
+
+static void fill_coef_job(const mpmc_hip_ctx *c, const SweepView &v, const DevAtoms &pa, const TholeParams &tp,
+                          const DirtyMoves &dm, int nt, const MoveList &m, CoefJob &cj) {
+    cj.pa = pa;
+    cj.tp = tp;
+    cj.dm = dm;
+    cj.nt = nt;
+    cj.ntld = v.ntld;
+    cj.C = v.C;
+    cj.m = m;
+    cj.gx = c->d_x;
+    cj.gy = c->d_y;
+    cj.gz = c->d_z;
+    cj.slot_of_atom = (const int *)v.d_slot;
+    cj.px = v.px;
+    cj.py = v.py;
+    cj.pz = v.pz;
 }
 
 static int print_inv_stamps(hipStream_t st, const unsigned long long *istamps, size_t nwg, int waves, const GsBuild &gb,
@@ -207,21 +291,7 @@
 
 static void hand_over_coef_job(mpmc_hip_ctx *c, const SweepView &v, const DevAtoms &pa, const TholeParams &tp,
                                const DirtyMoves &dm, int nt) {
-    CoefJob &cj = c->call.coef_job;
-    cj.pa = pa;
-    cj.tp = tp;
-    cj.dm = dm;
-    cj.nt = nt;
-    cj.ntld = v.ntld;
-    cj.C = v.C;
-    cj.m = c->pending;
-    cj.gx = c->d_x;
-    cj.gy = c->d_y;
-    cj.gz = c->d_z;
-    cj.slot_of_atom = (const int *)v.d_slot;
-    cj.px = v.px;
-    cj.py = v.py;
-    cj.pz = v.pz;
+    fill_coef_job(c, v, pa, tp, dm, nt, c->pending, c->call.coef_job);
     c->call.coef_job_valid = true;
     if (c->call.side_carry) c->call.side_moves = c->pending;
     c->pending.n = 0;
@@ -244,20 +314,13 @@
                            v.palpha, v.pflags);
         v.pos_valid = incremental && (&v == &c->view[0]);
     }
-    DevAtoms pa = a;
-    pa.x = v.px;
-    pa.y = v.py;
-    pa.z = v.pz;
-    pa.alpha = v.palpha;
-    pa.flags = v.pflags;
-    pa.n = v.nv;
-    pa.npad = v.nvpad;
+    const DevAtoms pa = view_atoms(a, v);
     const TholeParams tp = thole_params(c, v.d_idx);
     ScopedTimer t(c, T_AMAT, st);
     DirtyList dl;
     int nd = 0;
     const bool can_update = incremental && !c->all_dirty && c->opt.incremental && collect_dirty_slots(c, v, dl, nd);
-    const int nt = std::max(1, (v.nv + kCoefTile - 1) / kCoefTile);
+    const int nt = view_tiles(v);
     bool coef_updated = false;
     int tail = -1;
     if (v.rebuild_from >= 0) {
@@ -278,26 +341,7 @@
                                                           v.ntld, v.C));
             else if (nd > 0 && fuse_moves && nd <= kMaxDirtyMoves) {
                 DirtyMoves dm;
-                dm.n = nd;
-                for (int k = 0; k < kMaxDirtyMoves; ++k) {
-                    dm.slot[k] = (k < nd) ? dl.slot[k] : 0;
-                    dm.x[k] = dm.y[k] = dm.z[k] = 0.0;
-                }
-                bool all_found = true;
-                for (int k = 0; k < nd; ++k) {
-                    const int atom = v.h_idx[dl.slot[k]];
-                    bool found = false;
-                    for (int e = 0; e < c->pending.n; ++e) {
-                        if (c->pending.idx[e] == atom) {
-                            dm.x[k] = c->pending.x[e];
-                            dm.y[k] = c->pending.y[e];
-                            dm.z[k] = c->pending.z[e];
-                            found = true;
-                        }
-                    }
-                    all_found &= found;
-                }
-                if (all_found) {
+                if (fill_dirty_moves(v, dl.slot, nd, c->pending, dm)) {
                     hand_over_coef_job(c, v, pa, tp, dm, nt);
                     if (want_chain && launch_coef_job(c, bx)) return -1;
                 } else {
@@ -426,7 +470,50 @@
     return nt * (nt + 1) / 2 + nt > c->num_cus;
 }
 
+static int enqueue_head_for_moves(mpmc_hip_ctx *c, const MoveList &m, bool &done) {
+    done = false;
+    const SweepView &v = c->view[0];
+    if (!(v.C_valid && v.pos_valid && c->field_part_valid) || m.n <= 0 || m.n > kMaxMoves) return 0;
+    const FieldPlan plan = field_plan(c);
+    if (plan.mode == kFieldEwald || c->field_key != plan.key) return 0;
+    DirtyBlocks sel;
+    if (!blocks_of(std::vector<int>(m.idx, m.idx + m.n), sel)) return 0;
+    int slots[kMaxDirty], nd = 0;
+    if (!slots_of(v, m.idx, m.n, slots, nd) || nd == 0 || nd > kMaxDirtyMoves) return 0;
+    DirtyMoves dm;
+    if (!fill_dirty_moves(v, slots, nd, m, dm)) return 0;
+    const DevAtoms a = dev_atoms(c);
+    const DevBox bx = dev_box(c);
+    CoefJob cj;
+    fill_coef_job(c, v, view_atoms(a, v), thole_params(c, v.d_idx), dm, view_tiles(v), m, cj);
+    dim3 grid = field_grid(plan, sel);
+    if (!coef_job_fits(grid, sel, cj)) return 0;
+    grid.z = 3;
+    const int mode = plan.mode;
+    MPMC_LAUNCH_HEAD(c, grid, a, bx, plan.fp, sel, cj);
+    done = true;
+    return 0;
+}
+
+static int cancel_prefetch(mpmc_hip_ctx *c) {
+    if (!c->pf.outstanding) return 0;
+    c->pf.outstanding = false;
+    ++c->pf_cancelled;
+    HIPCHK(hipSetDevice(c->device));
+    bool done = false;
+    if (enqueue_head_for_moves(c, c->pf.old, done)) return -1;
+    if (!done) {
+        SweepView &v0 = c->view[0];
+        hipLaunchKernelGGL(apply_moves_kernel, dim3(1), dim3(64), 0, c->stream, c->pf.old, c->d_x, c->d_y, c->d_z,
+                           (const int *)v0.d_slot, v0.px, v0.py, v0.pz);
+        c->all_dirty = true;
+    }
+    c->main_writes = true;
+    return 0;
+}
+
 static int complete_pending_sweep(mpmc_hip_ctx *c) {
+    if (cancel_prefetch(c)) return -1;
     if (c->psweep.sweeps.empty()) return 0;
     PendingSweep p;
     std::swap(p, c->psweep);
diff --git a/mpmc_amd/csrc/step_plan.h b/mpmc_amd/csrc/step_plan.h
--- a/mpmc_amd/csrc/step_plan.h
+++ b/mpmc_amd/csrc/step_plan.h
@@ -35,6 +35,34 @@
             return false;
         }
         out.blk[out.n++] = b;
+    }
+    return true;
+}
+
+static inline int move_index(const MoveList &m, int atom) {
+    for (int e = 0; e < m.n; ++e)
+        if (m.idx[e] == atom) return e;
+    return -1;
+}
+static inline bool same_moves(const MoveList &a, const MoveList &b) {
+    if (a.n != b.n || a.n < 0 || a.n > kMaxMoves) return false;
+    const size_t nb = (size_t)a.n * sizeof(double);
+    return memcmp(a.idx, b.idx, (size_t)a.n * sizeof(int)) == 0 && memcmp(a.x, b.x, nb) == 0 && memcmp(a.y, b.y, nb) == 0 &&
+           memcmp(a.z, b.z, nb) == 0;
+}
+static inline bool prefetch_is_used(const MoveList &pending, const MoveList &prefetched, const std::vector<int> &dirty_atoms,
+                                    bool all_dirty, unsigned long long rev_now, unsigned long long rev_then) {
+    if (all_dirty || rev_now != rev_then || prefetched.n <= 0 || !same_moves(pending, prefetched)) return false;
+    for (int atom : dirty_atoms)
+        if (move_index(prefetched, atom) < 0) return false;
+    return true;
+}
+static inline bool prefetch_is_covered(const MoveList &pending, const MoveList &prefetched) {
+    for (int e = 0; e < prefetched.n; ++e) {
+        const int k = move_index(pending, prefetched.idx[e]);
+        if (k < 0 || memcmp(&pending.x[k], &prefetched.x[e], sizeof(double)) || memcmp(&pending.y[k], &prefetched.y[e], sizeof(double)) ||
+            memcmp(&pending.z[k], &prefetched.z[e], sizeof(double)))
+            return false;
     }
     return true;
 }
diff --git a/mpmc_amd/csrc/step_pods.h b/mpmc_amd/csrc/step_pods.h
--- a/mpmc_amd/csrc/step_pods.h
+++ b/mpmc_amd/csrc/step_pods.h
@@ -6,6 +6,13 @@
 struct DirtyBlocks {
     int n;
     int blk[kMaxDirtyBlocks];
+};
+
+constexpr int kMaxMoves = 32;
+struct MoveList {
+    int n;
+    int idx[kMaxMoves];
+    double x[kMaxMoves], y[kMaxMoves], z[kMaxMoves];
 };
 
 struct SweepParams {
diff --git a/mpmc_amd/engine.py b/mpmc_amd/engine.py
--- a/mpmc_amd/engine.py
+++ b/mpmc_amd/engine.py
@@ -18,6 +18,7 @@
     "mpmc_hip_set_exact_polar", "mpmc_hip_get_polarizability_tensor", "mpmc_hip_set_thole_model",
     "mpmc_hip_update_atoms", "mpmc_hip_insert_molecule", "mpmc_hip_remove_molecule", "mpmc_hip_edit_molecules",
     "mpmc_hip_slot_count", "mpmc_hip_set_sweep_order", "mpmc_hip_energy", "mpmc_hip_energy_begin", "mpmc_hip_energy_end",
+    "mpmc_hip_prefetch_atoms",
     "mpmc_hip_download_dipoles",
     "mpmc_hip_download_amatrix", "mpmc_hip_download_ranking", "mpmc_hip_get_timings",
     "mpmc_hip_comm_unique_id", "mpmc_hip_comm_create", "mpmc_hip_comm_size", "mpmc_hip_comm_rank",
@@ -97,6 +98,10 @@
         ("resident_calls", C.c_int),
         ("resident_fallbacks", C.c_int),
         ("pending_sweeps", C.c_int),
+        ("prefetch_issued", C.c_int),
+        ("prefetch_used", C.c_int),
+        ("prefetch_overwritten", C.c_int),
+        ("prefetch_cancelled", C.c_int),
     ]
 
 
@@ -201,6 +206,7 @@
     lib.mpmc_hip_energy.argtypes = [vp, C.POINTER(Result)]
     lib.mpmc_hip_energy_begin.argtypes = [vp]
     lib.mpmc_hip_energy_end.argtypes = [vp, C.POINTER(Result)]
+    lib.mpmc_hip_prefetch_atoms.argtypes = [vp, C.c_int, C.c_int, vp, vp, vp]
     lib.mpmc_hip_download_dipoles.argtypes = [vp, vp, vp, vp, vp]
     lib.mpmc_hip_download_amatrix.argtypes = [vp, vp]
     lib.mpmc_hip_download_ranking.argtypes = [vp, vp, vp]
@@ -508,6 +514,14 @@
     def energy_begin(self):
         _chk(self.lib.mpmc_hip_energy_begin(self.ctx))
 
+    def prefetch_atoms(self, first, pos):
+        pos = np.ascontiguousarray(pos, dtype=np.float64)
+        cols = [np.ascontiguousarray(pos[:, k]) for k in range(3)]
+        rc = self.lib.mpmc_hip_prefetch_atoms(self.ctx, int(first), pos.shape[0], *[a.ctypes.data for a in cols])
+        if rc < 0:
+            _chk(rc)
+        return rc == 1
+
     def energy_end(self):
         r = Result()
         _chk(self.lib.mpmc_hip_energy_end(self.ctx, C.byref(r)))
diff --git a/mpmc_amd/host.py b/mpmc_amd/host.py
--- a/mpmc_amd/host.py
+++ b/mpmc_amd/host.py
@@ -68,6 +68,12 @@
     lib.host_force_volume_move.restype = None
     lib.host_init_chain_no_energy.argtypes = [vp]
     lib.host_init_chain_no_energy.restype = None
+    lib.host_predict_next.argtypes = [vp, vp, C.c_int, C.POINTER(C.c_int)]
+    lib.host_decide_and_move.argtypes = [vp, C.c_int]
+    lib.host_decide_and_move.restype = None
+    lib.host_get_altered.argtypes = [vp, C.POINTER(C.c_int)]
+    lib.make_move.argtypes = [vp]
+    lib.make_move.restype = None
     lib.host_get_disp_flags.argtypes = [vp, vp]
     lib.host_get_disp_flags.restype = None
     lib.host_get_dispersion.argtypes = [vp, vp, vp, vp]
@@ -273,6 +279,27 @@
         self.lib.host_get_sync_counts(self.ptr, out)
         return dict(full_uploads=int(out[0]), edit_calls=int(out[1]), molecules_edited=int(out[2]))
 
+    def predict_next(self, cap=32):
+        xyz = np.zeros((cap, 3))
+        idx = C.c_int(-1)
+        n = self.lib.host_predict_next(self.ptr, xyz.ctypes.data, int(cap), C.byref(idx))
+        return (idx.value, xyz[:n].copy()) if n > 0 else None
+
+    def decide_and_move(self, accept):
+        self.lib.host_decide_and_move(self.ptr, int(bool(accept)))
+
+    def altered(self):
+        rank = C.c_int(-1)
+        return self.lib.host_get_altered(self.ptr, C.byref(rank)), rank.value
+
+    def mc_steps_trace(self, nsteps):
+        trace = np.zeros((int(nsteps), 6))
+        self.lib.host_mc_steps_trace.argtypes = [C.c_void_p, C.c_int, C.c_void_p]
+        r = self.lib.host_mc_steps_trace(self.ptr, int(nsteps), trace.ctypes.data)
+        if r < 0:
+            raise engine.EngineError(engine.load().mpmc_hip_last_error().decode())
+        return trace
+
     def mc_steps(self, nsteps):
         r = self.lib.host_mc_steps(self.ptr, int(nsteps))
         if r < 0:
diff --git a/mpmc_amd/host/energy_hip.c b/mpmc_amd/host/energy_hip.c
--- a/mpmc_amd/host/energy_hip.c
+++ b/mpmc_amd/host/energy_hip.c
@@ -143,6 +143,13 @@
     shim_state *st = state_of(system, 0);
     if (st) *out = st->tsum;
     else memset(out, 0, sizeof(*out));
+    if (st && st->ctx) {
+        mpmc_hip_timings t;
+        if (!mpmc_hip_get_timings(st->ctx, &t)) {
+            out->prefetch_issued = t.prefetch_issued; out->prefetch_used = t.prefetch_used;
+            out->prefetch_overwritten = t.prefetch_overwritten; out->prefetch_cancelled = t.prefetch_cancelled;
+        }
+    }
 }
 
 static double g_prof[4];
@@ -1081,6 +1088,25 @@
     return 0;
 }
 
+int energy_hip_prefetch_displacement(system_t *system, molecule_t *molecule, const double *xyz) {
+    shim_state *st = state_of(system, 0);
+    if (!st || !st->ctx || !st->in_sync || !molecule) return 0;
+    int i = -1;
+    for (int k = 0; k < st->nres; k++)
+        if (st->res[k].mol == molecule) {
+            i = k;
+            break;
+        }
+    if (i < 0 || st->res[i].frozen) return 0;
+    const int n = st->res[i].natoms;
+    double x[32], y[32], z[32];
+    if (n <= 0 || n > 32 || natoms_of(molecule) != n) return 0;
+    for (int k = 0; k < n; k++) {
+        x[k] = xyz[3 * k + 0]; y[k] = xyz[3 * k + 1]; z[k] = xyz[3 * k + 2];
+    }
+    return mpmc_hip_prefetch_atoms(st->ctx, st->res[i].slot, n, x, y, z);
+}
+
 double energy_hip_end(system_t *system) {
     shim_state *st = state_of(system, 0);
     if (!st || !st->ctx) return NAN;
diff --git a/mpmc_amd/host/energy_hip.h b/mpmc_amd/host/energy_hip.h
--- a/mpmc_amd/host/energy_hip.h
+++ b/mpmc_amd/host/energy_hip.h
@@ -12,6 +12,8 @@
 double energy_hip_end(system_t *system);
 int energy_hip_failed(system_t *system);
 const char *energy_hip_unsupported(const system_t *system);
+
+int energy_hip_prefetch_displacement(system_t *system, molecule_t *molecule, const double *xyz);
 
 void energy_hip_note_moved(system_t *system, molecule_t *now, molecule_t *was);
 void energy_hip_note_list_changed(system_t *system);
diff --git a/mpmc_amd/host/mc.c b/mpmc_amd/host/mc.c
--- a/mpmc_amd/host/mc.c
+++ b/mpmc_amd/host/mc.c
@@ -395,6 +395,55 @@
             }
     }
     checkpoint(system);
+}
+
+#define PREDICT_MAX_ATOMS 32
+int predict_next_displacement(system_t *system, molecule_t **which, double *xyz, int cap) {
+    const checkpoint_t *cp = system->checkpoint;
+    if (system->ensemble != ENSEMBLE_NVT || system->cavity_bias || !system->movable_valid || !system->rng_initialized) return 0;
+    if (!cp || cp->movetype != MOVETYPE_DISPLACE) return 0;
+    if (cap > PREDICT_MAX_ATOMS) cap = PREDICT_MAX_ATOMS;
+    unsigned int saved_mt[624];
+    memcpy(saved_mt, system->rng_mt, sizeof(saved_mt));
+    const int saved_mti = system->rng_mti;
+    int natoms = 0;
+    (void)get_rand(system);
+    const int altered = (int)floor(get_rand(system) * system->observables->N);
+    molecule_t *pick = (altered >= 0 && altered < system->nmovable) ? system->movable[altered] : NULL;
+    if (pick && altered != cp->altered_index && pick != cp->molecule_altered && pick != cp->molecule_backup) {
+        for (const atom_t *a = pick->atoms; a; a = a->next) natoms++;
+        if (natoms > cap) natoms = 0;
+    }
+    if (natoms > 0) {
+        atom_t atoms[PREDICT_MAX_ATOMS];
+        molecule_t scratch;
+        int k = 0;
+        for (const atom_t *a = pick->atoms; a; a = a->next, k++) {
+            atoms[k].mass = a->mass;
+            for (int p = 0; p < 3; p++) atoms[k].pos[p] = a->pos[p];
+            atoms[k].next = (k + 1 < natoms) ? &atoms[k + 1] : NULL;
+        }
+        scratch.atoms = atoms;
+        scratch.next = NULL;
+        update_com(&scratch);
+        translate(system, &scratch, system->pbc, system->move_factor);
+        rotate(system, &scratch, system->pbc, system->rot_factor);
+        for (k = 0; k < natoms; k++)
+            for (int p = 0; p < 3; p++) xyz[3 * k + p] = atoms[k].pos[p];
+        *which = pick;
+    }
+    memcpy(system->rng_mt, saved_mt, sizeof(saved_mt));
+    system->rng_mti = saved_mti;
+    return natoms;
+}
+
+double energy_of_trial(system_t *system, int prefetch_next) {
+    if (!system->hip || !prefetch_next) return energy(system);
+    if (energy_hip_begin(system)) return NAN;
+    molecule_t *next = NULL;
+    double xyz[3 * PREDICT_MAX_ATOMS];
+    if (predict_next_displacement(system, &next, xyz, PREDICT_MAX_ATOMS) > 0) energy_hip_prefetch_displacement(system, next, xyz);
+    return energy_hip_end(system);
 }
 
 void boltzmann_factor(system_t *system, double initial_energy, double final_energy) {
@@ -512,7 +561,7 @@
     for (system->step = 1; system->step <= system->numsteps; (system->step)++) {
         initial_energy = system->observables->energy;
         make_move(system);
-        final_energy = energy(system);
+        final_energy = energy_of_trial(system, system->step < system->numsteps);
         if (energy_hip_failed(system)) {
             error("MC: the device engine failed, stopping the chain\n");
             free(rcv);
diff --git a/mpmc_amd/host/mpmc_host.h b/mpmc_amd/host/mpmc_host.h
--- a/mpmc_amd/host/mpmc_host.h
+++ b/mpmc_amd/host/mpmc_host.h
@@ -158,6 +158,8 @@
 void restore(system_t *system);
 void make_move(system_t *system);
 void boltzmann_factor(system_t *system, double initial_energy, double final_energy);
+int predict_next_displacement(system_t *system, molecule_t **which, double *xyz, int cap);
+double energy_of_trial(system_t *system, int prefetch_next);
 void update_nodestats(nodestats_t *nodestats, avg_nodestats_t *avg_nodestats);
 void clear_avg_nodestats(system_t *system);
 void update_root_nodestats(system_t *system, avg_nodestats_t *avg_nodestats, avg_observables_t *avg_observables);
```

New measurement: 13490 MC steps/s. -3.7%, worse.
